# GaryGky/IDEAL-NeRF

Hardware: AMD Instinct MI355X
Metric: ray-samples/sec (64+128 pts, 512x512), whole job (higher is better)
Workload: dtype f32

## Files before the change

ideal-nerf_amd/csrc/idn_internal.h:

```cpp
#pragma once
#include <hip/hip_runtime.h>
#include <mutex>
#include <stdint.h>
#include <stddef.h>
#include "../../include/idealnerf.h"

namespace idn {

constexpr int kFragBytes = 1024;
constexpr int kFragFloats = 256;
constexpr int kSliceFrags = 64;
constexpr int kRingSlots = 2;
constexpr int kRingFrags = kRingSlots * kSliceFrags;
constexpr int kSliceBytes = kSliceFrags * kFragBytes;

constexpr int kNumLayers = 12;
constexpr int kLayerNT[kNumLayers] = {8, 8, 8, 8, 8, 8, 8, 8, 5, 4, 4, 1};
constexpr int kLayerKG[kNumLayers] = {8, 32, 32, 32, 32, 40, 32, 32, 36, 16, 16, 16};

constexpr int layer_f0(int l) {
    int f = 0;
    for (int i = 0; i < l; ++i) f += kLayerNT[i] * kLayerKG[i];
    return f;
}
constexpr int kUsedFrags = layer_f0(kNumLayers);
constexpr int kNumSlices =
    ((kUsedFrags + kSliceFrags - 1) / kSliceFrags + kRingSlots - 1) / kRingSlots * kRingSlots;
constexpr int kStreamFrags = kNumSlices * kSliceFrags;
static_assert(kUsedFrags == 2244, "layer table changed");
static_assert(kNumSlices % kRingSlots == 0, "slot of a slice must be static across passes");
static_assert(kRingFrags == 128, "FragReader addresses the ring as two 64-fragment halves");

constexpr int plain_f0(int l) {
    int f = 0;
    for (int i = 0; i < l; ++i) f += kLayerNT[i] * (kLayerKG[i] / 2);
    return f;
}
constexpr int kPlainUsedFrags = plain_f0(kNumLayers);
constexpr int kPlainNumSlices =
    ((kPlainUsedFrags + kSliceFrags - 1) / kSliceFrags + kRingSlots - 1) / kRingSlots * kRingSlots;
constexpr int kPlainStreamFrags = kPlainNumSlices * kSliceFrags;
static_assert(kPlainUsedFrags == 1122 && kPlainUsedFrags % 2 == 0, "plain stream table changed");

constexpr int kX6KFrags = 3;
constexpr int kX6SliceFrags = 16 * kX6KFrags;
constexpr int kX6RingFrags = kRingSlots * kX6SliceFrags;
constexpr int kX6UsedFrags = kX6KFrags * kPlainUsedFrags;
constexpr int kX6NumSlices = 2 * kNumSlices;
constexpr int kX6StreamFrags = kX6NumSlices * kX6SliceFrags;
static_assert(kX6UsedFrags <= kX6StreamFrags && kX6StreamFrags - kX6UsedFrags < kX6RingFrags + kX6SliceFrags, "x6 stream table");

constexpr int bias_off(int l) {
    int o = 0;
    for (int i = 0; i < l; ++i) o += kLayerNT[i] * 32;
    return o;
}
constexpr int kAlphaOff = bias_off(kNumLayers);
constexpr int kRgbOff = kAlphaOff + 256;
constexpr int kBiasFloats = kRgbOff + 3 * 128;
static_assert(kBiasFloats == 3136, "bias table changed");

constexpr int kSigmaChannel = 128;

enum { kActX0 = 0, kActDir = 1, kActA1 = 2, kActV1 = 10, kActCount = 13 };
constexpr int act_width(int i) { return i < 2 ? 64 : (i < kActV1 ? 256 : 128); }
constexpr int act_off(int i) {
    int o = 0;
    for (int k = 0; k < i; ++k) o += act_width(k);
    return o;
}
constexpr int kActCols = act_off(kActCount);
static_assert(kActCols == 2560, "activation slab layout changed");
constexpr int kMaskLayers = 11;
constexpr int kMaskFloatsPerPoint = kMaskLayers * 8;
constexpr int kActColsAll = kActCols + kMaskFloatsPerPoint;
__host__ __device__ inline size_t mask_index(int id, int64_t p_pad, int64_t wave_tile, int lane) {
    return ((size_t)id * (size_t)(p_pad / 32) + (size_t)wave_tile) * 64 + (size_t)lane;
}

int fail(int code, const char* fmt, ...);
#define IDN_HIP_CHECK(expr)                                                                   \
    do {                                                                                      \
        hipError_t _e = (expr);                                                               \
        if (_e != hipSuccess) return ::idn::fail(IDN_EHIP, "%s: %s", #expr, hipGetErrorString(_e)); \
    } while (0)

struct LaunchSetup {
    static constexpr int kMaxDevices = 64;
    std::mutex mu;
    int cus[kMaxDevices] = {};
    template <class OptIn>
    int get(OptIn&& opt_in, int* num_cu) {
        int dev = 0;
        IDN_HIP_CHECK(hipGetDevice(&dev));
        if (dev < 0 || dev >= kMaxDevices) return ::idn::fail(IDN_EUNSUPPORTED, "device index %d out of range", dev);
        std::lock_guard<std::mutex> lock(mu);
        if (!cus[dev]) {
            hipDeviceProp_t prop;
            IDN_HIP_CHECK(hipGetDeviceProperties(&prop, dev));
            if (int e = opt_in()) return e;
            cus[dev] = prop.multiProcessorCount;
        }
        *num_cu = cus[dev];
        return IDN_OK;
    }
};

struct ProfScope {
    int slot;
    hipStream_t s;
    ProfScope(hipStream_t s, int64_t points, int kind = IDN_PROF_MLP_FWD);
    ~ProfScope();
};

int launch_pack_f32(const idn_facenerf_params& p, float* packed, hipStream_t s);
int launch_pack_bf16x3(const idn_facenerf_params& p, float* packed, hipStream_t s, int fmt = 0);
int launch_pack_bf16x6(const idn_facenerf_params& p, float* packed, hipStream_t s);
int launch_mlp_bf16x6(const float* packed, const float* folded, const float* x, const float* rays, const float* z,
                      const float* pts, const float* dirs, int64_t n_points, int n_samples, float* raw, hipStream_t s,
                      float* acts = nullptr, int64_t p_pad = 0);
int launch_pack_bf16(const idn_facenerf_params& p, float* packed, hipStream_t s);
int launch_mlp_bf16(const float* packed, const float* folded, const float* x, const float* rays, const float* z,
                    const float* pts, const float* dirs, int64_t n_points, int n_samples, float* raw, hipStream_t s);
int launch_mlp_bf16x3(const float* packed, const float* folded, const float* x, const float* rays, const float* z,
                      const float* pts, const float* dirs, int64_t n_points, int n_samples, float* raw, hipStream_t s);
int launch_mlp_fp16x3(const float* packed, const float* folded, const float* x, const float* rays, const float* z,
                      const float* pts, const float* dirs, int64_t n_points, int n_samples, float* raw, hipStream_t s);
int launch_mlp(int precision, const float* packed, const float* folded, const float* x, const float* rays,
               const float* z, const float* pts, const float* dirs, int64_t n_points, int n_samples, float* raw,
               hipStream_t s);
int launch_fold(const idn_facenerf_params& p, const float* aud, const float* expr, const float* latent,
                float* folded, hipStream_t s);
int launch_mlp_f32(const float* packed, const float* folded, const float* x, const float* rays, const float* z,
                   const float* pts, const float* dirs, int64_t n_points, int n_samples, float* raw, hipStream_t s,
                   float* acts = nullptr, int64_t p_pad = 0);

int launch_frame_rays(const float* c2w, int H, int W, float focal, float cx, float cy, float near_, float far_,
                      int row0, int nrows, float* rays_out, hipStream_t s);
int launch_frame_rays_pixels(const float* c2w_host, int H, int W, float focal, float cx, float cy, float near_, float far_,
                             int64_t pix0, int npix, float* rays_out, hipStream_t s);
size_t audio_net_saved_floats(int n);
int launch_audio_net_fwd(const idn_audio_net_params* p, const float* windows, int n, float* out, float* saved, hipStream_t s);
int launch_audio_net_bwd(const idn_audio_net_params* p, const idn_audio_net_grads* g, const float* windows, const float* saved,
                         const float* d_out, int n, hipStream_t s);
int launch_to8b(const float* rgb, int64_t n_pixels, int swap_rb, unsigned char* out, int* flag, hipStream_t s);
int launch_compose_to8b(const float* head, const float* lw, const float* fg, int64_t n_pixels, int swap_rb,
                        unsigned char* out, unsigned char* fg_out, int* flag, hipStream_t s);
struct Draws {
    unsigned long long seed;
    long ray0;
    int on;
};
int launch_philox_uniform(unsigned long long seed, int which, int64_t row0, int64_t n_rows, int n_cols, float* out, hipStream_t s);
int launch_coarse_depths(const float* rays, const float* t_vals, const float* t_rand, int64_t n_rays, int S,
                         int lindisp, float* z, hipStream_t s, Draws draws = Draws{0, 0, 0});
int launch_composite(const float* raw, const float* z, const float* rays, const float* bc, int64_t n_rays, int S,
                     const float* noise, int white_bkgd, const idn_composite_out& out, hipStream_t s);
int launch_march(const float* raw, const float* z, const float* rays, const float* bc, const float* noise, int white_bkgd,
                 const idn_composite_out& out, const float* u, int u_per_ray, int64_t n_rays, int S, int Ni,
                 float* z_samples, int64_t* inds, float* cdf_out, float* z_fine, float* z_std, hipStream_t s,
                 Draws draws = Draws{0, 0, 0});
int launch_render_fused(int arrangement, const float* packed_c, const float* folded_c, const float* packed_f, const float* folded_f,
                        const float* rays, const float* bc, const float* z_c, float* z_f, const float* u, int u_per_ray, int64_t n_rays,
                        int white_bkgd, const idn_composite_out& co, const idn_composite_out& fo, float* z_std, float* tap_raw_c,
                        float* tap_raw_f, float* tap_z_fine, int64_t* tap_inds, float* tap_z_samples, float* tap_cdf, hipStream_t s,
                        Draws draws = Draws{0, 0, 0});
int launch_sample_pdf(const float* z, const float* weights, const float* cdf_in, const float* bins_in,
                      const float* u, int u_per_ray, int64_t n_rays, int S, int Ni, float* z_samples,
                      int64_t* inds, float* cdf_out, float* z_fine, float* z_std, hipStream_t s);

constexpr int kBwdStages = 11;
constexpr int kBwdNT[kBwdStages] = {4, 4, 4, 8, 8, 8, 8, 8, 8, 8, 8};
constexpr int kBwdKG[kBwdStages] = {2, 16, 16, 18, 32, 32, 32, 32, 32, 32, 32};
constexpr int kBwdHeadFrags = 280, kBwdTrunk0 = 384;
constexpr int bwd_f0(int s) {
    if (s >= 4) return kBwdTrunk0 + 256 * (s - 4);
    int f = 0;
    for (int i = 0; i < s; ++i) f += kBwdNT[i] * kBwdKG[i];
    return f;
}
static_assert(bwd_f0(3) + kBwdNT[3] * kBwdKG[3] == kBwdHeadFrags, "head stages");
constexpr int kBwdStreamFrags = kBwdTrunk0 + 7 * 256;
static_assert(kBwdStreamFrags % kSliceFrags == 0 && kBwdTrunk0 % kRingFrags == 0, "ring phase of the trunk stages");
constexpr int kBwdNumSlices = kBwdStreamFrags / kSliceFrags;

int launch_pack_f32_bwd(const idn_facenerf_params& p, float* packed_bwd, hipStream_t s);
int launch_delta_chain(const float* packed_bwd, const float* acts, int64_t p_pad, const float* d_rgb, float* dv0,
                       float* dv2, float* dv1, float* const da[8], hipStream_t s);
size_t bwd_stream_floats_x6();
int launch_pack_bf16x6_bwd(const idn_facenerf_params& p, float* packed_bwd, hipStream_t s);
int launch_delta_chain_x6(const float* packed_bwd, const float* acts, int64_t p_pad, const float* d_rgb, float* dv0,
                          float* dv2, float* dv1, float* const da[8], hipStream_t s);
size_t bwd_workspace_bytes(int64_t n_points);
size_t dw_gemm_workspace_bytes();
int launch_dw_gemm(const float* delta, int ld_delta, const float* acts, int ld_acts, int64_t rows, float* dW, float* db, int pipe,
                   void* ws, size_t ws_bytes, hipStream_t s);
int launch_pass_bwd(const idn_facenerf_params& p, const idn_facenerf_grads& gr, const float* aud, const float* expr,
                    const float* latent, const float* acts, const float* raw, const float* z, const float* rays,
                    const float* bc, int64_t n_rays, int S, const float* g_rgb, const float* g_fg, const float* g_lw,
                    const float* g_acc, float* d_aud, float* d_latent, void* ws, size_t ws_bytes, hipStream_t s);
int launch_facenerf_bwd(const idn_facenerf_params& p, const idn_facenerf_grads& gr, const float* aud, const float* expr,
                        const float* latent, const float* acts, int64_t n, const float* g_out, float* d_x, float* d_aud,
                        float* d_expr, float* d_latent, void* ws, size_t ws_bytes, hipStream_t s);

}
```

ideal-nerf_amd/csrc/mlp_f32_bwd.hip:

```cpp
#include "mlp_x6.h"

namespace idn {

__device__ __forceinline__ f32x16 mfma_b(float a, float b, f32x16 c) {
    return __builtin_amdgcn_mfma_f32_32x32x2f32(a, b, c, 0, 0, 0);
}

struct BwdPackStage {
    const float* w;
    const float* extra;
    int ld, col0, rows, cols, extra_at;
};
struct BwdPackDesc {
    BwdPackStage st[kBwdStages];
};
__global__ void pack_f32_bwd_kernel(BwdPackDesc d, float4* out) {
    const int gid = blockIdx.x * blockDim.x + threadIdx.x;
    if (gid >= kBwdStreamFrags * 64) return;
    const int f = gid >> 6, lane = gid & 63;
    float v[4] = {0.f, 0.f, 0.f, 0.f};
    int s = -1;
    for (int i = 0; i < kBwdStages; ++i)
        if (f >= bwd_f0(i) && f < bwd_f0(i) + kBwdNT[i] * kBwdKG[i]) s = i;
    if (s >= 0) {
        const BwdPackStage& S = d.st[s];
        const int rel = f - bwd_f0(s), t = rel / kBwdKG[s], g = rel - t * kBwdKG[s];
        const int n = 32 * t + (lane & 31);
        for (int j = 0; j < 4; ++j) {
            const int k = 8 * g + 4 * (lane >> 5) + j;
            if (n < S.cols) {
                if (k < S.rows) v[j] = S.w[(long)k * S.ld + S.col0 + n];
                else if (S.extra && k == S.extra_at) v[j] = S.extra[n];
            }
        }
    }
    out[gid] = make_float4(v[0], v[1], v[2], v[3]);
}

static void fill_bwd_desc(const idn_facenerf_params& p, BwdPackDesc& d) {
    const int C = p.dim_aud + p.dim_expr + p.dim_latent;
    d.st[0] = {p.rgb_w, nullptr, IDN_W / 2, 0, 3, IDN_W / 2, -1};
    d.st[1] = {p.views_w[2], nullptr, IDN_W / 2, 0, IDN_W / 2, IDN_W / 2, -1};
    d.st[2] = {p.views_w[1], nullptr, IDN_W / 2, 0, IDN_W / 2, IDN_W / 2, -1};
    d.st[3] = {p.views_w[0], p.alpha_w, IDN_W + IDN_VIEWS_CH + p.dim_expr, 0, IDN_W / 2, IDN_W, kSigmaChannel};
    for (int l = 7; l >= 1; --l) {
        BwdPackStage& S = d.st[4 + (7 - l)];
        S = {p.pts_w[l], nullptr, l == 5 ? IDN_PTS_CH + C + IDN_W : IDN_W, l == 5 ? IDN_PTS_CH + C : 0, IDN_W, IDN_W, -1};
    }
}

int launch_pack_f32_bwd(const idn_facenerf_params& p, float* packed_bwd, hipStream_t s) {
    BwdPackDesc d;
    fill_bwd_desc(p, d);
    const int total = kBwdStreamFrags * 64;
    hipLaunchKernelGGL(pack_f32_bwd_kernel, dim3((total + 255) / 256), dim3(256), 0, s, d, reinterpret_cast<float4*>(packed_bwd));
    IDN_HIP_CHECK(hipGetLastError());
    return IDN_OK;
}

struct DeltaArgs {
    const float* wstream;
    const float* acts;
    long p_pad;
    const float* d_rgb;
    float* dv0;
    float* dv2;
    float* dv1;
    float* da[8];
};

template <int F0, int NT, int KG, bool LAST, class BGet, class Side>
__device__ __forceinline__ void run_stage(f32x16 (&out)[NT], BGet&& bget, WStream& ws, FragReader& fr, Side&& side) {
    constexpr int STEPS = KG / 2, NP = NT * STEPS;
    static_assert(KG % 2 == 0 && F0 % 2 == 0, "fragments are consumed in pairs");
    if constexpr (F0 % kSliceFrags == 0) {
        ws.open_slice();
        fr.pref0 = fr.template issue<F0>();
        fr.pref1 = fr.template issue<F0 + 1>();
    }
    f32x4 a0 = fr.pref0, a1 = fr.pref1;
    static_for<NP>([&](auto PI) {
        constexpr int pi = decltype(PI)::value;
        constexpr int t = pi / STEPS, s = pi % STEPS, g0 = 2 * s, g1 = g0 + 1;
        constexpr int f = F0 + 2 * pi;
        constexpr bool next_crosses = ((f + 2) % kSliceFrags == 0);
        f32x4 n0 = a0, n1 = a1;
        if constexpr (!next_crosses && !(LAST && pi + 1 == NP)) {
            n0 = fr.template issue<f + 2>();
            n1 = fr.template issue<f + 3>();
            FragReader::retire<2>(a0, a1);
        } else {
            FragReader::retire<0>(a0, a1);
        }
        ws.template step_piece<f>();
        side(ic<t>{}, ic<s>{}, ic<0>{});
        out[t] = mfma_b(a0.x, bget(ic<g0>{}, ic<0>{}), out[t]);
        out[t] = mfma_b(a0.y, bget(ic<g0>{}, ic<1>{}), out[t]);
        out[t] = mfma_b(a0.z, bget(ic<g0>{}, ic<2>{}), out[t]);
        out[t] = mfma_b(a0.w, bget(ic<g0>{}, ic<3>{}), out[t]);
        out[t] = mfma_b(a1.x, bget(ic<g1>{}, ic<0>{}), out[t]);
        out[t] = mfma_b(a1.y, bget(ic<g1>{}, ic<1>{}), out[t]);
        out[t] = mfma_b(a1.z, bget(ic<g1>{}, ic<2>{}), out[t]);
        out[t] = mfma_b(a1.w, bget(ic<g1>{}, ic<3>{}), out[t]);
        if constexpr (next_crosses && pi + 1 < NP) {
            ws.open_slice();
            n0 = fr.template issue<f + 2>();
            n1 = fr.template issue<f + 3>();
        }
        a0 = n0;
        a1 = n1;
    });
    fr.pref0 = a0;
    fr.pref1 = a1;
}

template <int NT, int STEPS, int LD>
struct MaskSide {
    static constexpr bool kShadowStore = STEPS >= 8;
    f32x16* out;
    const uint32_t* mk;
    __amdgpu_buffer_rsrc_t rsrc;
    uint32_t voff;
    float* stage;
    float* rb;
    uint32_t raddr;
    int m, h;
    template <int T>
    __device__ __forceinline__ void apply(ic<T>) const {
        const uint32_t w = mk[T >> 1];
        static_for<16>([&](auto R) {
            constexpr int r = decltype(R)::value, i = 16 * (T & 1) + r;
            const int off = (int)(w << i) >> 31;
            out[T][r] = __uint_as_float(__float_as_uint(out[T][r]) & ~(uint32_t)off);
        });
    }
    template <int T>
    __device__ __forceinline__ void scatter(ic<T>) const {
        static_for<16>([&](auto R) {
            constexpr int r = decltype(R)::value;
            stage[m * kStagePitch + (r & 3) + 8 * (r >> 2) + 4 * h] = out[T][r];
        });
        asm volatile("" ::: "memory");
    }
    template <int Q>
    __device__ __forceinline__ void rows_read(ic<Q>) const {
        static_for<4>([&](auto I) {
            constexpr int i = decltype(I)::value;
            asm volatile("ds_read_b32 %0, %1 offset:%2" : "=v"(rb[i]) : "v"(raddr), "n"(2 * (4 * Q + i) * kStagePitch * 4) : "memory");
        });
    }
    template <int T, int Q>
    __device__ __forceinline__ void rows_store(ic<T>, ic<Q>) const {
        asm volatile("" : "+v"(rb[0]), "+v"(rb[1]), "+v"(rb[2]), "+v"(rb[3]));
        static_for<4>([&](auto I) {
            constexpr int i = decltype(I)::value;
            __builtin_amdgcn_raw_buffer_store_b32(__builtin_bit_cast(unsigned, rb[i]), rsrc, voff, (2 * (4 * Q + i) * LD + 32 * T) * 4, 0);
        });
    }
    template <int T>
    __device__ __forceinline__ void flush_tile(ic<T>) const {
        scatter(ic<T>{});
        static_for<4>([&](auto Q) {
            rows_read(Q);
            asm volatile("s_waitcnt lgkmcnt(0)" : "+v"(rb[0]), "+v"(rb[1]), "+v"(rb[2]), "+v"(rb[3])::"memory");
            rows_store(ic<T>{}, Q);
        });
    }
    __device__ __forceinline__ void finish() const {
        apply(ic<NT - 1>{});
        if constexpr (kShadowStore) flush_tile(ic<NT - 1>{});
        else static_for<NT>([&](auto T) { flush_tile(T); });
    }
    template <int T, int S, int H>
    __device__ __forceinline__ void operator()(ic<T>, ic<S>, ic<H>) const {
        constexpr int kApplyStep = STEPS > 1 ? 1 : 0;
        if constexpr (S == kApplyStep && T > 0) apply(ic<T - 1>{});
        if constexpr (kShadowStore && T > 0) {
            if constexpr (S == 2) scatter(ic<T - 1>{});
            if constexpr (S >= 4 && S <= 7) rows_store(ic<T - 1>{}, ic<S - 4>{});
            if constexpr (S >= 3 && S <= 6) rows_read(ic<S - 3>{});
        }
    }
};

template <int NT>
__device__ __forceinline__ void zero_tiles(f32x16 (&t)[NT]) {
    static_for<NT>([&](auto T) {
        static_for<16>([&](auto R) { t[decltype(T)::value][decltype(R)::value] = 0.0f; });
    });
}

constexpr int kDeltaLds = kRingFrags * kFragBytes + 4 * kStageFloats * 4;

__global__ __launch_bounds__(256, 1) void delta_chain_kernel(DeltaArgs a) {
    extern __shared__ __attribute__((aligned(16))) char smem[];
    char* ring = smem;
    const int tid = threadIdx.x, lane = tid & 63;
    const int wave = __builtin_amdgcn_readfirstlane(tid >> 6);
    const int m = lane & 31, h = lane >> 5;
    float* stage = reinterpret_cast<float*>(smem + kRingFrags * kFragBytes) + wave * kStageFloats;

    WStream ws;
    ws.init(a.wstream, kBwdNumSlices, ring, tid, wave);
    FragReader fr;
    fr.addr0 = (uint32_t)(uintptr_t)(__attribute__((address_space(3))) char*)ring + lane * 16;
    fr.addr1 = fr.addr0 + 64 * kFragBytes;
    const long ntiles = a.p_pad >> 7;
    const uint32_t raddr = (uint32_t)(uintptr_t)(__attribute__((address_space(3))) float*)stage + (h * kStagePitch + m) * 4;

    for (long tile = blockIdx.x; tile < ntiles; tile += gridDim.x) {
        const long p0 = tile * 128 + wave * 32;
        const long P = p0 + m;
        const f32x4 drgb = *reinterpret_cast<const f32x4*>(a.d_rgb + P * 64);
        const float dsig = a.dv0[P * 256 + kSigmaChannel];

        f32x16 A[8], B[8];
        float rb[4];
        typedef uint32_t u32x4 __attribute__((ext_vector_type(4)));
        const u32x4* mbase = reinterpret_cast<const u32x4*>(a.acts + (size_t)kActCols * a.p_pad);
        auto mask_load = [&](int id) { return mbase[mask_index(id, a.p_pad, tile * 4 + wave, lane)]; };
        u32x4 mask_nxt = mask_load(10);
        auto tiles_get = [](f32x16* arr) {
            return [arr](auto G, auto J) {
                constexpr int g = decltype(G)::value, j = decltype(J)::value;
                return arr[g >> 2][(g & 3) * 4 + j];
            };
        };
        auto stage_run = [&](auto Sc, auto F0c, auto LASTc, auto LDc, auto& out, auto&& bget, int next_id, float* dst) {
            constexpr int S = decltype(Sc)::value, F0 = decltype(F0c)::value;
            constexpr int NT = kBwdNT[S], KG = kBwdKG[S];
            zero_tiles<NT>(out);
            constexpr int LD = decltype(LDc)::value;
            const u32x4 mv = mask_nxt;
            const uint32_t mk[4] = {mv.x, mv.y, mv.z, mv.w};
            if (next_id >= 0) mask_nxt = mask_load(next_id);
            const MaskSide<NT, KG / 2, LD> side{&out[0], mk, rows_rsrc(dst + p0 * LD, LD), (uint32_t)((h * LD + m) * 4), stage, rb, raddr, m, h};
            run_stage<F0, NT, KG, decltype(LASTc)::value != 0>(out, bget, ws, fr, side);
            side.finish();
        };
        f32x16(&A4)[4] = reinterpret_cast<f32x16(&)[4]>(A);
        f32x16(&B4)[4] = reinterpret_cast<f32x16(&)[4]>(B);

        stage_run(ic<0>{}, ic<bwd_f0(0)>{}, ic<0>{}, ic<256>{}, A4,
                  [&](auto G, auto J) {
                      constexpr int g = decltype(G)::value, j = decltype(J)::value;
                      if constexpr (g == 0 && j < 3) return h ? 0.0f : drgb[j];
                      else return 0.0f;
                  },
                  9, a.dv2);
        stage_run(ic<1>{}, ic<bwd_f0(1)>{}, ic<0>{}, ic<256>{}, B4, tiles_get(A), 8, a.dv1);
        stage_run(ic<2>{}, ic<bwd_f0(2)>{}, ic<0>{}, ic<256>{}, A4, tiles_get(B), 7, a.dv0);
        stage_run(ic<3>{}, ic<bwd_f0(3)>{}, ic<1>{}, ic<256>{}, B,
                  [&](auto G, auto J) {
                      constexpr int g = decltype(G)::value, j = decltype(J)::value;
                      if constexpr (g < 16) return A[g >> 2][(g & 3) * 4 + j];
                      else if constexpr (g == 16 && j == 0) return h ? 0.0f : dsig;
                      else return 0.0f;
                  },
                  6, a.da[7]);
        finish_pass<kBwdHeadFrags, kBwdTrunk0>(ws);
#pragma unroll 1
        for (int l = 7; l >= 3; l -= 2) {
            stage_run(ic<4>{}, ic<bwd_f0(4)>{}, ic<0>{}, ic<256>{}, A, tiles_get(B), l - 2, a.da[l - 1]);
            stage_run(ic<5>{}, ic<bwd_f0(5)>{}, ic<0>{}, ic<256>{}, B, tiles_get(A), l - 3, a.da[l - 2]);
        }
        stage_run(ic<10>{}, ic<bwd_f0(10)>{}, ic<1>{}, ic<256>{}, A, tiles_get(B), -1, a.da[0]);
    }
    __builtin_amdgcn_s_waitcnt(0);
    __syncthreads();
}

int launch_delta_chain(const float* packed_bwd, const float* acts, int64_t p_pad, const float* d_rgb, float* dv0,
                       float* dv2, float* dv1, float* const da[8], hipStream_t s) {
    if (p_pad <= 0) return IDN_OK;
    if (p_pad % 128) return fail(IDN_EINVAL, "delta chain: p_pad %lld is not a multiple of 128", (long long)p_pad);
    static LaunchSetup setup;
    int num_cu = 0;
    if (int e = setup.get([]() -> int {
            IDN_HIP_CHECK(hipFuncSetAttribute(reinterpret_cast<const void*>(&delta_chain_kernel),
                                              hipFuncAttributeMaxDynamicSharedMemorySize, kDeltaLds));
            return IDN_OK;
        }, &num_cu))
        return e;
    const int64_t ntiles = p_pad / 128;
    const int grid = (int)(ntiles < num_cu ? ntiles : num_cu);
    DeltaArgs a{packed_bwd, acts, (long)p_pad, d_rgb, dv0, dv2, dv1, {}};
    for (int l = 0; l < 8; ++l) a.da[l] = da[l];
    ProfScope prof(s, p_pad, IDN_PROF_DELTA_CHAIN);
    hipLaunchKernelGGL(delta_chain_kernel, dim3(grid), dim3(256), kDeltaLds, s, a);
    IDN_HIP_CHECK(hipGetLastError());
    return IDN_OK;
}


constexpr int bwd6_f0(int s) { return kX6KFrags * (bwd_f0(s) / 2); }
constexpr int kBwd6StreamFrags = kX6KFrags * (kBwdStreamFrags / 2);
constexpr int kBwd6NumSlices = kBwd6StreamFrags / kX6SliceFrags;
static_assert(kBwd6StreamFrags % kX6SliceFrags == 0 && kBwd6NumSlices % kRingSlots == 0 && bwd6_f0(4) % kX6RingFrags == 0, "ring phase of the trunk stages");

__global__ void pack_bf16x6_bwd_kernel(BwdPackDesc d, uint4* out) {
    const int gid = blockIdx.x * blockDim.x + threadIdx.x;
    if (gid >= kBwd6StreamFrags * 64) return;
    const int f = gid >> 6, lane = gid & 63, part = f % kX6KFrags;
    unsigned w[4] = {0u, 0u, 0u, 0u};
    int s = -1;
    for (int i = 0; i < kBwdStages; ++i)
        if (f >= bwd6_f0(i) && f < bwd6_f0(i) + kX6KFrags * kBwdNT[i] * (kBwdKG[i] / 2)) s = i;
    if (s >= 0) {
        const BwdPackStage& S = d.st[s];
        const int ksn = kBwdKG[s] / 2;
        const int rel = (f - bwd6_f0(s)) / kX6KFrags, t = rel / ksn, ks = rel - t * ksn;
        const int n = 32 * t + (lane & 31), h = lane >> 5;
        for (int j = 0; j < 8; ++j) {
            const int k = 16 * ks + (j & 3) + 8 * (j >> 2) + 4 * h;
            float v = 0.f;
            if (n < S.cols) {
                if (k < S.rows) v = S.w[(long)k * S.ld + S.col0 + n];
                else if (S.extra && k == S.extra_at) v = S.extra[n];
            }
            const unsigned u1 = __float_as_uint(v);
            const unsigned p1 = (u1 + 0x7fffu + ((u1 >> 16) & 1u)) >> 16;
            const float r1 = v - __uint_as_float(p1 << 16);
            const unsigned u2 = __float_as_uint(r1);
            const unsigned p2 = (u2 + 0x7fffu + ((u2 >> 16) & 1u)) >> 16;
            const float r2 = r1 - __uint_as_float(p2 << 16);
            const unsigned u3 = __float_as_uint(r2);
            const unsigned p3 = (u3 + 0x7fffu + ((u3 >> 16) & 1u)) >> 16;
            const unsigned bits = part == 0 ? p1 : (part == 1 ? p2 : p3);
            w[j >> 1] |= bits << (16 * (j & 1));
        }
    }
    out[gid] = make_uint4(w[0], w[1], w[2], w[3]);
}

static_assert(kBwd6StreamFrags >= kBwdStreamFrags, "the six-piece stream is the larger of the two");
size_t bwd_stream_floats_x6() { return (size_t)kBwd6StreamFrags * kFragFloats; }

int launch_pack_bf16x6_bwd(const idn_facenerf_params& p, float* packed_bwd, hipStream_t s) {
    BwdPackDesc d;
    fill_bwd_desc(p, d);
    const int total = kBwd6StreamFrags * 64;
    hipLaunchKernelGGL(pack_bf16x6_bwd_kernel, dim3((total + 255) / 256), dim3(256), 0, s, d, reinterpret_cast<uint4*>(packed_bwd));
    IDN_HIP_CHECK(hipGetLastError());
    return IDN_OK;
}

namespace x6 {

template <int F0, int NT, int KS, bool LAST, int OPEN_YOUNGER, int MID_YOUNGER, class BGet, class Side>
__device__ __forceinline__ void run_stage6(f32x16* O, BGet&& bget, WStream6& ws, FragReader& fr, f32x4 (&pref)[3], Side&& side) {
    constexpr int NP = NT * KS;
    static_assert(F0 % kX6KFrags == 0, "triples");
    static_for<NT>([&](auto T) { static_for<16>([&](auto R) { O[decltype(T)::value][decltype(R)::value] = 0.0f; }); });
    if constexpr (F0 % kX6SliceFrags == 0) {
        ws.template open_slice<OPEN_YOUNGER>();
        static_for<3>([&](auto Q) { pref[decltype(Q)::value] = issue6<F0 + decltype(Q)::value>(fr); });
        retire3<0>(pref);
    }
    f32x4 a[3] = {pref[0], pref[1], pref[2]};
    static_for<NP>([&](auto PI) {
        constexpr int pi = decltype(PI)::value;
        constexpr int t = pi / KS, s = pi % KS;
        constexpr int f = F0 + kX6KFrags * pi;
        constexpr bool next_crosses = ((f + kX6KFrags) % kX6SliceFrags == 0);
        constexpr bool has_next = !(LAST && pi + 1 == NP);
        f32x4 n[3] = {a[0], a[1], a[2]};
        if constexpr (!next_crosses && has_next) {
            static_for<3>([&](auto Q) { n[decltype(Q)::value] = issue6<f + kX6KFrags + decltype(Q)::value>(fr); });
            if constexpr (pi > 0) retire3<3>(a);
        } else {
            if constexpr (pi > 0) retire3<0>(a);
        }
        step_pieces6<f>(ws);
        const f32x4 b1 = bget(ic<0>{}, ic<s>{}), b2 = bget(ic<1>{}, ic<s>{}), b3 = bget(ic<2>{}, ic<s>{});
        O[t] = mfma_bf(a[0], b1, O[t]);
        O[t] = mfma_bf(a[0], b2, O[t]);
        O[t] = mfma_bf(a[1], b1, O[t]);
        O[t] = mfma_bf(a[1], b2, O[t]);
        side(ic<t>{}, ic<s>{});
        O[t] = mfma_bf(a[0], b3, O[t]);
        O[t] = mfma_bf(a[2], b1, O[t]);
        if constexpr (next_crosses && pi + 1 < NP) {
            ws.template open_slice<(t >= 1 ? MID_YOUNGER : 0)>();
            static_for<3>([&](auto Q) { n[decltype(Q)::value] = issue6<f + kX6KFrags + decltype(Q)::value>(fr); });
        }
        a[0] = n[0];
        a[1] = n[1];
        a[2] = n[2];
    });
    if constexpr (!LAST && (F0 + kX6KFrags * NP) % kX6SliceFrags != 0) retire3<0>(a);
    pref[0] = a[0];
    pref[1] = a[1];
    pref[2] = a[2];
}

template <int KS>
struct MaskStoreSide {
    f32x16* O;
    const uint32_t* mk;
    float* row;
    template <int T>
    __device__ __forceinline__ void apply(ic<T>) const {
        const uint32_t w = mk[T >> 1];
        static_for<16>([&](auto R) {
            constexpr int r = decltype(R)::value, i = 16 * (T & 1) + r;
            const int off = (int)(w << i) >> 31;
            O[T][r] = __uint_as_float(__float_as_uint(O[T][r]) & ~(uint32_t)off);
        });
    }
    template <int T, int Q0>
    __device__ __forceinline__ void store2(ic<T>, ic<Q0>) const {
        static_for<2>([&](auto I) {
            constexpr int q = Q0 + decltype(I)::value;
            *reinterpret_cast<f32x4*>(row + 32 * T + 8 * q) = f32x4{O[T][4 * q], O[T][4 * q + 1], O[T][4 * q + 2], O[T][4 * q + 3]};
        });
    }
    template <int T>
    __device__ __forceinline__ void whole(ic<T>) const {
        apply(ic<T>{});
        store2(ic<T>{}, ic<0>{});
        store2(ic<T>{}, ic<2>{});
    }
    template <int T, int Q>
    __device__ __forceinline__ void store1(ic<T>, ic<Q>) const {
        *reinterpret_cast<f32x4*>(row + 32 * T + 8 * Q) = f32x4{O[T][4 * Q], O[T][4 * Q + 1], O[T][4 * Q + 2], O[T][4 * Q + 3]};
    }
    template <int T, int S>
    __device__ __forceinline__ void operator()(ic<T>, ic<S>) const {
        if constexpr (KS == 16 && T > 0) {
            if constexpr (S == 7) apply(ic<T - 1>{});
            if constexpr (S >= 8 && S < 16 && (S & 1) == 0) store1(ic<T - 1>{}, ic<(S - 8) / 2>{});
        }
    }
};

constexpr int kDelta6Lds = kX6RingFrags * kFragBytes;

__global__ __launch_bounds__(256, 1) void delta_chain_x6_kernel(DeltaArgs a) {
    extern __shared__ __attribute__((aligned(16))) char smem[];
    char* ring = smem;
    const int tid = threadIdx.x, lane = tid & 63;
    const int wave = __builtin_amdgcn_readfirstlane(tid >> 6);
    const int m = lane & 31, h = lane >> 5;

    WStream6 ws;
    ws.init(a.wstream, kBwd6NumSlices, ring, tid, wave);
    FragReader fr;
    fr.addr0 = (uint32_t)(uintptr_t)(__attribute__((address_space(3))) char*)ring + lane * 16;
    fr.addr1 = fr.addr0 + 64 * kFragBytes;
    const long ntiles = a.p_pad >> 7;
    f32x4 pref[3] = {{0.f, 0.f, 0.f, 0.f}, {0.f, 0.f, 0.f, 0.f}, {0.f, 0.f, 0.f, 0.f}};

    for (long tile = blockIdx.x; tile < ntiles; tile += gridDim.x) {
        const long P = tile * 128 + wave * 32 + m;
        const f32x4 drgb = *reinterpret_cast<const f32x4*>(a.d_rgb + P * 64);
        const float dsig = a.dv0[P * 256 + kSigmaChannel];
        f32x4 in_rgb[3], in_sig[3];
        {
            const f32x4 z4 = {0.f, 0.f, 0.f, 0.f};
            float r[3][2], g[3];
            split3(h ? 0.0f : drgb[0], h ? 0.0f : drgb[1], r[0][0], r[1][0], r[2][0]);
            split3(h ? 0.0f : drgb[2], 0.0f, r[0][1], r[1][1], r[2][1]);
            float unused0, unused1, unused2;
            (void)unused0; (void)unused1; (void)unused2;
            split3(h ? 0.0f : dsig, 0.0f, g[0], g[1], g[2]);
            static_for<3>([&](auto Q) {
                constexpr int q = decltype(Q)::value;
                in_rgb[q] = z4;
                in_rgb[q][0] = r[q][0];
                in_rgb[q][1] = r[q][1];
                in_sig[q] = z4;
                in_sig[q][0] = g[q];
            });
        }

        settle(in_rgb);
        settle(in_sig);
        PTile6 Pt[8];
        f32x16 O[8];
        typedef uint32_t u32x4 __attribute__((ext_vector_type(4)));
        const u32x4* mbase = reinterpret_cast<const u32x4*>(a.acts + (size_t)kActCols * a.p_pad);
        auto mask_load = [&](int id) { return mbase[mask_index(id, a.p_pad, tile * 4 + wave, lane)]; };
        u32x4 mask_nxt = mask_load(10);
        auto tiles = [&](auto Q, auto S_) {
            constexpr int q = decltype(Q)::value, s = decltype(S_)::value;
            return Pt[s >> 1].p[q][s & 1];
        };
        auto stage_run = [&](auto F0c, auto NTc, auto KSc, auto LASTc, auto LDc, auto YOUNGERc, auto&& bget, int next_id, float* dst) __attribute__((always_inline)) {
            constexpr int NT = decltype(NTc)::value, LD = decltype(LDc)::value;
            const u32x4 mv = mask_nxt;
            const uint32_t mk[4] = {mv.x, mv.y, mv.z, mv.w};
            if (next_id >= 0) mask_nxt = mask_load(next_id);
            const MaskStoreSide<decltype(KSc)::value> side{O, mk, dst + P * LD + 4 * h};
            constexpr bool trunk = decltype(F0c)::value >= bwd6_f0(4);
            run_stage6<decltype(F0c)::value, NT, decltype(KSc)::value, decltype(LASTc)::value != 0, decltype(YOUNGERc)::value, (trunk ? 4 : 0)>(O, bget, ws, fr, pref, side);
            if constexpr (trunk) side.whole(ic<NT - 1>{});
            else static_for<NT>([&](auto T) { side.whole(T); });
            static_for<NT>([&](auto T) { convert_tile<false>(O[decltype(T)::value], Pt[decltype(T)::value]); });
        };
        stage_run(ic<bwd6_f0(0)>{}, ic<4>{}, ic<1>{}, ic<0>{}, ic<256>{}, ic<0>{}, [&](auto Q, auto) { return in_rgb[decltype(Q)::value]; }, 9, a.dv2);
        stage_run(ic<bwd6_f0(1)>{}, ic<4>{}, ic<8>{}, ic<0>{}, ic<256>{}, ic<0>{}, tiles, 8, a.dv1);
        stage_run(ic<bwd6_f0(2)>{}, ic<4>{}, ic<8>{}, ic<0>{}, ic<256>{}, ic<0>{}, tiles, 7, a.dv0);
        stage_run(ic<bwd6_f0(3)>{}, ic<8>{}, ic<9>{}, ic<1>{}, ic<256>{}, ic<0>{},
                  [&](auto Q, auto S_) {
                      constexpr int q = decltype(Q)::value, s = decltype(S_)::value;
                      if constexpr (s < 8) return Pt[s >> 1].p[q][s & 1];
                      else return in_sig[q];
                  },
                  6, a.da[7]);
        finish_pass6<kX6KFrags * (kBwdHeadFrags / 2), bwd6_f0(4)>(ws);
        stage_run(ic<bwd6_f0(4)>{}, ic<8>{}, ic<16>{}, ic<0>{}, ic<256>{}, ic<0>{}, tiles, 5, a.da[6]);
#pragma unroll 1
        for (int L = 6; L >= 2; --L)
            stage_run(ic<bwd6_f0(5)>{}, ic<8>{}, ic<16>{}, ic<0>{}, ic<256>{}, ic<8>{}, tiles, L - 2, a.da[L - 1]);
        stage_run(ic<bwd6_f0(10)>{}, ic<8>{}, ic<16>{}, ic<1>{}, ic<256>{}, ic<8>{}, tiles, -1, a.da[0]);
    }
    __builtin_amdgcn_s_waitcnt(0);
    __syncthreads();
}

}

int launch_delta_chain_x6(const float* packed_bwd, const float* acts, int64_t p_pad, const float* d_rgb, float* dv0,
                          float* dv2, float* dv1, float* const da[8], hipStream_t s) {
    if (p_pad <= 0) return IDN_OK;
    if (p_pad % 128) return fail(IDN_EINVAL, "delta chain: p_pad %lld is not a multiple of 128", (long long)p_pad);
    static LaunchSetup setup;
    int num_cu = 0;
    if (int e = setup.get([]() -> int {
            IDN_HIP_CHECK(hipFuncSetAttribute(reinterpret_cast<const void*>(&x6::delta_chain_x6_kernel),
                                              hipFuncAttributeMaxDynamicSharedMemorySize, x6::kDelta6Lds));
            return IDN_OK;
        }, &num_cu))
        return e;
    const int64_t ntiles = p_pad / 128;
    const int grid = (int)(ntiles < num_cu ? ntiles : num_cu);
    DeltaArgs a{packed_bwd, acts, (long)p_pad, d_rgb, dv0, dv2, dv1, {}};
    for (int l = 0; l < 8; ++l) a.da[l] = da[l];
    ProfScope prof(s, p_pad, IDN_PROF_DELTA_CHAIN_X6);
    hipLaunchKernelGGL(x6::delta_chain_x6_kernel, dim3(grid), dim3(256), x6::kDelta6Lds, s, a);
    IDN_HIP_CHECK(hipGetLastError());
    return IDN_OK;
}

}
```

ideal-nerf_amd/csrc/train.hip:

```cpp
#include "idn_internal.h"
#include <cstdlib>
#include <type_traits>

namespace idn {

typedef float f32x16 __attribute__((ext_vector_type(16)));
typedef float f32x4 __attribute__((ext_vector_type(4)));

__device__ __forceinline__ f32x16 mfma32(float a, float b, f32x16 c) {
    return __builtin_amdgcn_mfma_f32_32x32x2f32(a, b, c, 0, 0, 0);
}
__device__ __forceinline__ int d_row(int r, int hh) { return (r & 3) + 8 * (r >> 2) + 4 * hh; }

struct TNArgs {
    const float* A; int lda;
    const float* B; int ldb;
    float* part;
    int N, K;
    long P;
    int chunks_per_split;
    float* cpart;
    int b_split, b_off0, b_off1;
};

template <int N>
struct LdsVec;
template <>
struct LdsVec<4> {
    f32x4 v;
    template <int OFF>
    __device__ __forceinline__ void issue(uint32_t addr) { asm volatile("ds_read_b128 %0, %1 offset:%2" : "=v"(v) : "v"(addr), "n"(OFF) : "memory"); }
    __device__ __forceinline__ float get(int j) const { return v[j]; }
};
template <>
struct LdsVec<2> {
    typedef float f32x2 __attribute__((ext_vector_type(2)));
    f32x2 v;
    template <int OFF>
    __device__ __forceinline__ void issue(uint32_t addr) { asm volatile("ds_read_b64 %0, %1 offset:%2" : "=v"(v) : "v"(addr), "n"(OFF) : "memory"); }
    __device__ __forceinline__ float get(int j) const { return v[j]; }
};
template <>
struct LdsVec<1> {
    float v;
    template <int OFF>
    __device__ __forceinline__ void issue(uint32_t addr) { asm volatile("ds_read_b32 %0, %1 offset:%2" : "=v"(v) : "v"(addr), "n"(OFF) : "memory"); }
    __device__ __forceinline__ float get(int) const { return v; }
};
template <int OFF>
__device__ __forceinline__ void lds_read_f32(float& dst, uint32_t addr) {
    asm volatile("ds_read_b32 %0, %1 offset:%2" : "=v"(dst) : "v"(addr), "n"(OFF) : "memory");
}
__device__ __forceinline__ float landed(float& v) {
    asm volatile("" : "+v"(v));
    return v;
}
template <int NEWER, class VA, class VB>
__device__ __forceinline__ void lds_retire(VA& a, VB& b) {
    if constexpr (NEWER == 0) asm volatile("s_waitcnt lgkmcnt(0)" : "+v"(a.v), "+v"(b.v)::"memory");
    else asm volatile("s_waitcnt lgkmcnt(2)" : "+v"(a.v), "+v"(b.v)::"memory");
}
template <int N>
using ic_ = std::integral_constant<int, N>;
template <int N, class F>
__device__ __forceinline__ void tn_static_for(F&& f) {
    if constexpr (N > 0) {
        tn_static_for<N - 1>(f);
        f(std::integral_constant<int, N - 1>{});
    }
}

constexpr int kTnRows = 16, kTnBufs = 3;
constexpr int kTnNarrowBufs = 3;
constexpr int kTnRows4x1 = 32, kTnRowsThin = 64;
constexpr int kTnNarrowSplits = 256;

template <int NTW, int KTW, int NB = kTnBufs, int R = kTnRows>
__global__ __launch_bounds__(256) void gemm_tn_kernel(TNArgs g) {
    static_assert(R % 16 == 0, "chunks are multiples of 16 points");
    constexpr int NPA = NTW * R / 16, NPB = KTW * R / 16;
    static_assert(NB >= 3 && (NB - 2) * (NPA + NPB) <= 63, "vmcnt is a 6-bit field");
    constexpr int BN = 64 * NTW, BK = 64 * KTW;
    constexpr int kTileFloats = R * (BN + BK);
    constexpr int kSteps = R / 2;
    constexpr int NP = NPA + NPB;
    static_assert(NP <= kSteps, "at most one piece per step");
    extern __shared__ __attribute__((aligned(16))) float tn_smem[];
    const int tid = threadIdx.x, lane = tid & 63;
    const int w = __builtin_amdgcn_readfirstlane(tid >> 6);
    const int i = lane & 31, hh = lane >> 5;
    const int wr = w >> 1, wc = w & 1;
    const int n0 = blockIdx.x * BN, k0 = blockIdx.y * BK;
    const int split = blockIdx.z;
    f32x16 acc[NTW][KTW];
#pragma unroll
    for (int a = 0; a < NTW; ++a)
#pragma unroll
        for (int b = 0; b < KTW; ++b)
            for (int r = 0; r < 16; ++r) acc[a][b][r] = 0.f;

    const long c_begin = (long)split * g.chunks_per_split;
    long c_end = c_begin + g.chunks_per_split;
    const long c_total = g.P / R;
    if (c_end > c_total) c_end = c_total;
    const bool colsum_block = g.cpart != nullptr && blockIdx.y == 0;
    const bool do_colsum = colsum_block && tid < BN;
    const int ccol = tid < BN ? tid : 0;
    float csum = 0.0f;

    constexpr int kRowsPerPieceA = 256 / BN > 0 ? 256 / BN : 1, kRowsPerPieceB = 256 / BK > 0 ? 256 / BK : 1;
    const __amdgpu_buffer_rsrc_t rsrcA = __builtin_amdgcn_make_buffer_rsrc(const_cast<float*>(g.A + n0 + c_begin * R * (long)g.lda), 0, 0xfffffffc, 0x00020000);
    const __amdgpu_buffer_rsrc_t rsrcB = __builtin_amdgcn_make_buffer_rsrc(const_cast<float*>(g.B + k0 + c_begin * R * (long)g.ldb), 0, 0xfffffffc, 0x00020000);
    const uint32_t voffA = ((lane / (BN / 4)) * g.lda + (lane % (BN / 4)) * 4) * 4;
    const uint32_t voffB = ((lane / (BK / 4)) * g.ldb + (lane % (BK / 4)) * 4) * 4;
    const uint32_t rowA = g.lda * 4, rowB = g.ldb * 4;
    auto piece_a = [&](long c, int buf, int ja) {
        const int pc = NPA * w + ja;
        __builtin_amdgcn_raw_ptr_buffer_load_lds(rsrcA, (__attribute__((address_space(3))) void*)(tn_smem + buf * kTileFloats + pc * 256), 16, voffA,
                                                 (uint32_t)(((c - c_begin) * R + pc * kRowsPerPieceA) * rowA), 0, 0);
    };
    auto piece_b = [&](long c, int buf, int jb) {
        const int pc = NPB * w + jb;
        __builtin_amdgcn_raw_ptr_buffer_load_lds(rsrcB, (__attribute__((address_space(3))) void*)(tn_smem + buf * kTileFloats + R * BN + pc * 256), 16, voffB,
                                                 (uint32_t)(((c - c_begin) * R + pc * kRowsPerPieceB) * rowB), 0, 0);
    };
    auto piece = [&](long c, int buf, int j) {
        if (j < NPA) piece_a(c, buf, j);
        else if (j < NP) piece_b(c, buf, j - NPA);
    };
    const uint32_t smem0 = (uint32_t)(uintptr_t)(__attribute__((address_space(3))) float*)tn_smem;
    const uint32_t a_addr0 = smem0 + (hh * BN + NTW * (32 * wr + i)) * 4;
    const uint32_t b_addr0 = smem0 + (R * BN + hh * BK + KTW * (32 * wc + i)) * 4;
    for (int ahead = 0; ahead < NB - 1; ++ahead)
        for (int j = 0; j < NP; ++j) piece(c_begin + ahead < c_end ? c_begin + ahead : c_end - 1, ahead, j);
    int buf = 0;
    for (long c = c_begin; c < c_end; ++c) {
        asm volatile("s_waitcnt vmcnt(%0)" ::"n"((NB - 2) * NP) : "memory");
        __builtin_amdgcn_s_barrier();
        asm volatile("" ::: "memory");
        const int buf2 = buf >= 1 ? buf - 1 : NB - 1;
        const long cnext = c + NB - 1 < c_end ? c + NB - 1 : c_end - 1;
        float cs[16];
        auto cs_issue = [&](int batch) {
            const uint32_t caddr = smem0 + buf * (kTileFloats * 4) + ccol * 4 + batch * (16 * BN * 4);
            tn_static_for<16>([&](auto Row) {
                lds_read_f32<decltype(Row)::value * BN * 4>(cs[decltype(Row)::value], caddr);
            });
        };
        static_assert(R / 16 <= kSteps / 4, "one batch of column reads per iteration of the first half loop");
        if (colsum_block) cs_issue(0);
        LdsVec<NTW> a0v, a1v;
        LdsVec<KTW> b0v, b1v;
        constexpr int kStepA = 2 * BN * 4, kStepB = 2 * BK * 4;
        uint32_t pa = a_addr0 + buf * (kTileFloats * 4), pb = b_addr0 + buf * (kTileFloats * 4);
        a0v.template issue<0>(pa);
        b0v.template issue<0>(pb);
        static_assert(NPA <= kSteps / 2 && NPB <= kSteps / 2, "pieces of one matrix fit one half of a chunk");
        constexpr int M = NTW * KTW;
        if constexpr (M >= 4) {
            auto step = [&](LdsVec<NTW>& ca, LdsVec<KTW>& cb, auto&& side0, auto&& side1, auto&& side2) {
                lds_retire<0>(ca, cb);
                tn_static_for<M>([&](auto M_) {
                    constexpr int m = decltype(M_)::value, x = m / KTW, y = m % KTW;
                    acc[x][y] = mfma32(ca.get(x), cb.get(y), acc[x][y]);
                    if constexpr (m < 3) {
                        __builtin_amdgcn_sched_barrier(0);
                        if constexpr (m == 0) side0();
                        if constexpr (m == 1) side1();
                        if constexpr (m == 2) side2();
                        __builtin_amdgcn_sched_barrier(0);
                    }
                });
            };
#pragma unroll 1
            for (int it = 0; it < kSteps / 4; ++it) {
                step(a0v, b0v,
                     [&]() { a1v.template issue<kStepA>(pa); b1v.template issue<kStepB>(pb); },
                     [&]() { if (2 * it < NPA) piece_a(cnext, buf2, 2 * it); },
                     [&]() {
                         if (colsum_block && it < R / 16) {
                             tn_static_for<16>([&](auto Row) { csum += landed(cs[decltype(Row)::value]); });
                         }
                         pa += 2 * kStepA;
                         pb += 2 * kStepB;
                     });
                step(a1v, b1v,
                     [&]() { a0v.template issue<0>(pa); b0v.template issue<0>(pb); },
                     [&]() { if (2 * it + 1 < NPA) piece_a(cnext, buf2, 2 * it + 1); },
                     [&]() { if (colsum_block && it + 1 < R / 16) cs_issue(it + 1); });
            }
#pragma unroll 1
            for (int it = 0; it < kSteps / 4; ++it) {
                const bool last = it == kSteps / 4 - 1;
                step(a0v, b0v,
                     [&]() { a1v.template issue<kStepA>(pa); b1v.template issue<kStepB>(pb); },
                     [&]() { if (2 * it < NPB) piece_b(cnext, buf2, 2 * it); },
                     [&]() {
                         pa = last ? pa : pa + 2 * kStepA;
                         pb = last ? pb : pb + 2 * kStepB;
                     });
                step(a1v, b1v,
                     [&]() { a0v.template issue<0>(pa); b0v.template issue<0>(pb); },
                     [&]() { if (2 * it + 1 < NPB) piece_b(cnext, buf2, 2 * it + 1); },
                     [&]() {});
            }
        } else {
            static_assert(M == 2 && kSteps % 8 == 0, "the two-pair schedule");
            LdsVec<NTW> a2v, a3v;
            LdsVec<KTW> b2v, b3v;
            a1v.template issue<kStepA>(pa);
            b1v.template issue<kStepB>(pb);
            auto quad = [&](LdsVec<NTW>& c0a, LdsVec<KTW>& c0b, LdsVec<NTW>& c1a, LdsVec<KTW>& c1b, LdsVec<NTW>& n0a, LdsVec<KTW>& n0b,
                            LdsVec<NTW>& n1a, LdsVec<KTW>& n1b, bool last, auto&& side_c, auto&& side_d) {
                lds_retire<0>(c0a, c0b);
                lds_retire<0>(c1a, c1b);
                const uint32_t na = last ? pa : pa + 2 * kStepA, nb = last ? pb : pb + 2 * kStepB;
                auto mf = [&](LdsVec<NTW>& ca, LdsVec<KTW>& cb, auto M_) {
                    constexpr int m = decltype(M_)::value, x = m / KTW, y = m % KTW;
                    acc[x][y] = mfma32(ca.get(x), cb.get(y), acc[x][y]);
                    __builtin_amdgcn_sched_barrier(0);
                };
                mf(c0a, c0b, ic_<0>{});
                n0a.template issue<0>(na);
                n0b.template issue<0>(nb);
                __builtin_amdgcn_sched_barrier(0);
                mf(c0a, c0b, ic_<1>{});
                n1a.template issue<kStepA>(na);
                n1b.template issue<kStepB>(nb);
                __builtin_amdgcn_sched_barrier(0);
                mf(c1a, c1b, ic_<0>{});
                side_c();
                __builtin_amdgcn_sched_barrier(0);
                mf(c1a, c1b, ic_<1>{});
                side_d();
                pa = na;
                pb = nb;
                __builtin_amdgcn_sched_barrier(0);
            };
#pragma unroll 1
            for (int it = 0; it < kSteps / 8; ++it) {
                quad(a0v, b0v, a1v, b1v, a2v, b2v, a3v, b3v, false,
                     [&]() { if (2 * it < NPA) piece_a(cnext, buf2, 2 * it); },
                     [&]() {
                         if (colsum_block && it < R / 16) {
                             tn_static_for<16>([&](auto Row) { csum += landed(cs[decltype(Row)::value]); });
                         }
                     });
                quad(a2v, b2v, a3v, b3v, a0v, b0v, a1v, b1v, false,
                     [&]() { if (2 * it + 1 < NPA) piece_a(cnext, buf2, 2 * it + 1); },
                     [&]() { if (colsum_block && it + 1 < R / 16) cs_issue(it + 1); });
            }
#pragma unroll 1
            for (int it = 0; it < kSteps / 8; ++it) {
                quad(a0v, b0v, a1v, b1v, a2v, b2v, a3v, b3v, false,
                     [&]() { if (2 * it < NPB) piece_b(cnext, buf2, 2 * it); }, [&]() {});
                quad(a2v, b2v, a3v, b3v, a0v, b0v, a1v, b1v, it == kSteps / 8 - 1,
                     [&]() { if (2 * it + 1 < NPB) piece_b(cnext, buf2, 2 * it + 1); }, [&]() {});
            }
            lds_retire<0>(a1v, b1v);
        }
        lds_retire<0>(a0v, b0v);
        buf = buf + 1 == NB ? 0 : buf + 1;
    }
    asm volatile("s_waitcnt vmcnt(0)" ::: "memory");
    if (do_colsum) g.cpart[(long)split * g.N + n0 + tid] = csum;
    float* out = g.part + (long)split * g.N * g.K;
#pragma unroll
    for (int x = 0; x < NTW; ++x)
#pragma unroll
        for (int r = 0; r < 16; ++r) {
            const int n = n0 + NTW * (32 * wr + d_row(r, hh)) + x;
            float* dst = out + (long)n * g.K + k0 + KTW * (32 * wc + i);
            if constexpr (KTW == 4) {
                *reinterpret_cast<f32x4*>(dst) = f32x4{acc[x][0][r], acc[x][1][r], acc[x][2][r], acc[x][3][r]};
            } else {
#pragma unroll
                for (int y = 0; y < KTW; ++y) dst[y] = acc[x][y][r];
            }
        }
}

typedef __bf16 tn_bf16x8 __attribute__((ext_vector_type(8)));
typedef unsigned tn_u32x4 __attribute__((ext_vector_type(4)));
typedef int tn_i32x4 __attribute__((ext_vector_type(4)));
__device__ __forceinline__ f32x16 mfma_bf16(f32x4 a, f32x4 b, f32x16 c) {
    return __builtin_amdgcn_mfma_f32_32x32x16_bf16(__builtin_bit_cast(tn_bf16x8, a), __builtin_bit_cast(tn_bf16x8, b), c, 0, 0, 0);
}
__device__ __forceinline__ unsigned tn_cvt_pk_bf16(float x0, float x1) {
    unsigned r;
    asm("v_cvt_pk_bf16_f32 %0, %1, %2" : "=v"(r) : "v"(x0), "v"(x1));
    return r;
}
__device__ __forceinline__ void split3(float x0, float x1, unsigned& p1, unsigned& p2, unsigned& p3) {
    p1 = tn_cvt_pk_bf16(x0, x1);
    float r0 = x0 - __uint_as_float(p1 << 16), r1 = x1 - __uint_as_float(p1 & 0xffff0000u);
    p2 = tn_cvt_pk_bf16(r0, r1);
    r0 = r0 - __uint_as_float(p2 << 16);
    r1 = r1 - __uint_as_float(p2 & 0xffff0000u);
    p3 = tn_cvt_pk_bf16(r0, r1);
}
constexpr int kX6BufBytes = 2 * 8 * 3 * kFragBytes;
constexpr int kX6Lds = 2 * kX6BufBytes;

struct X6Frag {
    f32x4 v;
    template <int OFF>
    __device__ __forceinline__ void issue(uint32_t addr) { asm volatile("ds_read_b128 %0, %1 offset:%2" : "=v"(v) : "v"(addr), "n"(OFF) : "memory"); }
};
template <int N>
__device__ __forceinline__ void x6_retire(X6Frag (&f)[3]) {
    static_assert(N <= 15, "lgkmcnt is a 4-bit field");
    asm volatile("s_waitcnt lgkmcnt(%3)" : "+v"(f[0].v), "+v"(f[1].v), "+v"(f[2].v) : "n"(N) : "memory");
}

__device__ __forceinline__ void gemm_tn_x6_item(const TNArgs& g, const int split, char* x6_smem) {
    const int tid = threadIdx.x, lane = tid & 63;
    const int w = __builtin_amdgcn_readfirstlane(tid >> 6);
    const int i = lane & 31, hh = lane >> 5;
    const int wr = w >> 1, wc = w & 1;
    f32x16 acc[4][4];
#pragma unroll
    for (int a = 0; a < 4; ++a)
#pragma unroll
        for (int b = 0; b < 4; ++b)
            for (int r = 0; r < 16; ++r) acc[a][b][r] = 0.f;

    const long c_begin = (long)split * g.chunks_per_split;
    long c_end = c_begin + g.chunks_per_split;
    const long c_total = g.P / kTnRows;
    if (c_end > c_total) c_end = c_total;
    const int n_chunks = (int)(c_end - c_begin);
    auto make_rsrc = [](const float* ptr) {
        const uint64_t a64 = (uint64_t)(uintptr_t)ptr;
        return tn_i32x4{(int)(uint32_t)a64, (int)((uint32_t)(a64 >> 32) & 0xffffu), (int)0xfffffffcu, 0x00020000};
    };
    const tn_i32x4 rsrcA = make_rsrc(g.A + c_begin * kTnRows * (long)g.lda);
    const tn_i32x4 rsrcB = make_rsrc(g.B + c_begin * kTnRows * (long)g.ldb);
    const int voff = tid * 4;
    const int voffB = g.b_split ? (tid < 128 ? g.b_off0 : g.b_off1) + (tid & 127) * 4 : voff;
    const int rowA = g.lda * 4, rowB = g.ldb * 4;
    float ra[kTnRows], rb[kTnRows];
#pragma unroll
    for (int p = 0; p < kTnRows; ++p) ra[p] = rb[p] = 0.f;
    auto load_row_at = [&](float& dst, const tn_i32x4& rsrc, int soff, int vo) {
        asm volatile("buffer_load_dword %0, %1, %2, %3 offen" : "+v"(dst) : "v"(vo), "s"(rsrc), "s"(soff) : "memory");
    };
    auto load_row = [&](float& dst, const tn_i32x4& rsrc, int soff) { load_row_at(dst, rsrc, soff, voff); };
    auto load_chunk = [&](int rc) {
        const int base = (rc < n_chunks ? rc : n_chunks - 1) * kTnRows;
#pragma unroll
        for (int p = 0; p < kTnRows; ++p) load_row(ra[p], rsrcA, (base + p) * rowA);
#pragma unroll
        for (int p = 0; p < kTnRows; ++p) load_row_at(rb[p], rsrcB, (base + p) * rowB, voffB);
    };
    char* const my_slot = x6_smem + (tid >> 5) * (3 * kFragBytes) + (tid & 31) * 16;
    auto split_store = [&](int buf, int X, const float (&r)[kTnRows]) {
        unsigned pw[3][8];
#pragma unroll
        for (int j = 0; j < 8; ++j) split3(r[2 * j], r[2 * j + 1], pw[0][j], pw[1][j], pw[2][j]);
        char* dst = my_slot + buf * kX6BufBytes + X * (8 * 3 * kFragBytes);
#pragma unroll
        for (int q = 0; q < 3; ++q)
#pragma unroll
            for (int h2 = 0; h2 < 2; ++h2)
                *reinterpret_cast<tn_u32x4*>(dst + q * kFragBytes + h2 * 512) =
                    tn_u32x4{pw[q][4 * h2], pw[q][4 * h2 + 1], pw[q][4 * h2 + 2], pw[q][4 * h2 + 3]};
    };
    const bool do_colsum = g.cpart != nullptr;
    float csum = 0.0f, csum1 = 0.0f;
    auto colsum = [&]() {
        float s0 = (ra[0] + ra[1]) + (ra[2] + ra[3]), s1 = (ra[4] + ra[5]) + (ra[6] + ra[7]);
        float s2 = (ra[8] + ra[9]) + (ra[10] + ra[11]), s3 = (ra[12] + ra[13]) + (ra[14] + ra[15]);
        csum += (s0 + s1) + (s2 + s3);
    };
    const uint32_t smem0 = (uint32_t)(uintptr_t)(__attribute__((address_space(3))) char*)x6_smem;
    const uint32_t a_base = smem0 + (4 * wr) * (3 * kFragBytes) + lane * 16;
    const uint32_t b_base = smem0 + (8 + 4 * wc) * (3 * kFragBytes) + lane * 16;

    load_chunk(0);
#pragma unroll
    for (int p = 0; p < kTnRows; ++p) asm volatile("s_waitcnt vmcnt(0)" : "+v"(ra[p]), "+v"(rb[p])::"memory");
    colsum();
    split_store(0, 0, ra);
    split_store(0, 1, rb);
    load_chunk(1);
    asm volatile("s_waitcnt lgkmcnt(0)" ::: "memory");
    __builtin_amdgcn_s_barrier();
    asm volatile("" ::: "memory");

    X6Frag fa[4][3], fb[4][3];
    auto issue_first_row = [&](uint32_t pa, uint32_t pb) {
        tn_static_for<3>([&](auto Q) { fa[0][decltype(Q)::value].template issue<decltype(Q)::value * kFragBytes>(pa); });
        tn_static_for<2>([&](auto Y) {
            tn_static_for<3>([&](auto Q) {
                fb[decltype(Y)::value][decltype(Q)::value].template issue<(decltype(Y)::value * 3 + decltype(Q)::value) * kFragBytes>(pb);
            });
        });
    };
    issue_first_row(a_base, b_base);
#pragma unroll 1
    for (int rc = 0; rc < n_chunks; ++rc) {
        const int buf = rc & 1;
        const uint32_t pa = a_base + buf * kX6BufBytes, pb = b_base + buf * kX6BufBytes;
        tn_static_for<2>([&](auto Y) {
            tn_static_for<3>([&](auto Q) {
                fb[decltype(Y)::value + 2][decltype(Q)::value].template issue<((decltype(Y)::value + 2) * 3 + decltype(Q)::value) * kFragBytes>(pb);
            });
        });
        tn_static_for<3>([&](auto X) {
            tn_static_for<3>([&](auto Q) {
                fa[decltype(X)::value + 1][decltype(Q)::value].template issue<((decltype(X)::value + 1) * 3 + decltype(Q)::value) * kFragBytes>(pa);
            });
        });
        auto mm2 = [&](int x, int y0, int y1) {
#define X6_TERM(QA, QB)                                                   \
    acc[x][y0] = mfma_bf16(fa[x][QA].v, fb[y0][QB].v, acc[x][y0]);        \
    acc[x][y1] = mfma_bf16(fa[x][QA].v, fb[y1][QB].v, acc[x][y1]);
            X6_TERM(0, 0) X6_TERM(0, 1) X6_TERM(1, 0) X6_TERM(1, 1) X6_TERM(0, 2) X6_TERM(2, 0)
#undef X6_TERM
        };
        x6_retire<15>(fa[0]);
        x6_retire<15>(fb[0]);
        x6_retire<15>(fb[1]);
        mm2(0, 0, 1);
        x6_retire<9>(fb[2]);
        x6_retire<9>(fb[3]);
        mm2(0, 2, 3);
        x6_retire<0>(fa[1]);
        x6_retire<0>(fa[2]);
        x6_retire<0>(fa[3]);
        const unsigned live_mask = rc + 1 < n_chunks ? 0xffffffffu : 0u;
        const int nbase = (rc + 2 < n_chunks ? rc + 2 : n_chunks - 1) * kTnRows;
        char* const dst = my_slot + (buf ^ 1) * kX6BufBytes;
        unsigned pw[2][3][8];
        float t0 = 0.f, t1 = 0.f;
        auto slice = [&](auto X_, auto S_) {
            constexpr int X = decltype(X_)::value, sl = decltype(S_)::value;
            float (&r)[kTnRows] = *(X ? &rb : &ra);
            auto store = [&](auto Q_, auto H_) {
                constexpr int q = decltype(Q_)::value, h2 = decltype(H_)::value;
                *reinterpret_cast<tn_u32x4*>(dst + X * (8 * 3 * kFragBytes) + q * kFragBytes + h2 * 512) =
                    tn_u32x4{pw[X][q][4 * h2], pw[X][q][4 * h2 + 1], pw[X][q][4 * h2 + 2], pw[X][q][4 * h2 + 3]};
            };
            if constexpr (sl < 24) {
                constexpr int j = sl / 3, ph = sl % 3;
                if constexpr (ph == 0) {
                    asm volatile("s_waitcnt vmcnt(30)" : "+v"(r[2 * j]), "+v"(r[2 * j + 1])::"memory");
                    const unsigned p1 = tn_cvt_pk_bf16(r[2 * j], r[2 * j + 1]);
                    pw[X][0][j] = p1;
                    t0 = r[2 * j] - __uint_as_float(p1 << 16);
                    t1 = r[2 * j + 1] - __uint_as_float(p1 & 0xffff0000u);
                    if constexpr (X == 0) {
                        csum += __uint_as_float(__float_as_uint(r[2 * j]) & live_mask);
                        csum1 += __uint_as_float(__float_as_uint(r[2 * j + 1]) & live_mask);
                        asm volatile("" : "+v"(csum), "+v"(csum1));
                    }
                } else if constexpr (ph == 1) {
                    const unsigned p2 = tn_cvt_pk_bf16(t0, t1);
                    pw[X][1][j] = p2;
                    t0 = t0 - __uint_as_float(p2 << 16);
                    t1 = t1 - __uint_as_float(p2 & 0xffff0000u);
                    pw[X][2][j] = tn_cvt_pk_bf16(t0, t1);
                } else {
                    load_row_at(r[2 * j], X ? rsrcB : rsrcA, (nbase + 2 * j) * (X ? rowB : rowA), X ? voffB : voff);
                    load_row_at(r[2 * j + 1], X ? rsrcB : rsrcA, (nbase + 2 * j + 1) * (X ? rowB : rowA), X ? voffB : voff);
                    if constexpr (j >= 3 && j < 6) store(ic_<j - 3>{}, ic_<0>{});
                    if constexpr (j == 7) store(ic_<0>{}, ic_<1>{});
                }
            } else if constexpr (sl == 24) {
                store(ic_<1>{}, ic_<1>{});
            } else if constexpr (sl == 25) {
                store(ic_<2>{}, ic_<1>{});
            }
        };
        __builtin_amdgcn_sched_barrier(0);
        tn_static_for<72>([&](auto K_) {
            constexpr int k = decltype(K_)::value;
            constexpr int x = 1 + k / 24, kk = k % 24, y = 2 * (kk / 12) + (kk % 2), t = (kk % 12) / 2;
            constexpr int qa = t == 2 || t == 3 ? 1 : (t == 5 ? 2 : 0);
            constexpr int qb = t == 1 || t == 3 ? 1 : (t == 4 ? 2 : 0);
            acc[x][y] = mfma_bf16(fa[x][qa].v, fb[y][qb].v, acc[x][y]);
            constexpr int kX1 = 26;
            if constexpr (k < kX1) slice(ic_<0>{}, ic_<k>{});
            else slice(ic_<1>{}, ic_<k - kX1>{});
            if constexpr (k == 59) {
                asm volatile("s_waitcnt lgkmcnt(0)" ::: "memory");
                __builtin_amdgcn_s_barrier();
                asm volatile("" ::: "memory");
                issue_first_row(a_base + (buf ^ 1) * kX6BufBytes, b_base + (buf ^ 1) * kX6BufBytes);
            }
            __builtin_amdgcn_sched_barrier(0);
        });
    }
    x6_retire<0>(fa[0]);
    x6_retire<0>(fb[0]);
    x6_retire<0>(fb[1]);
#pragma unroll
    for (int p = 0; p < kTnRows; ++p) asm volatile("s_waitcnt vmcnt(0)" : "+v"(ra[p]), "+v"(rb[p])::"memory");
    if (do_colsum) g.cpart[(long)split * g.N + tid] = csum + csum1;
    float* out = g.part + (long)split * g.N * g.K;
#pragma unroll
    for (int x = 0; x < 4; ++x)
#pragma unroll
        for (int y = 0; y < 4; ++y)
#pragma unroll
            for (int r = 0; r < 16; ++r)
                out[(long)(32 * (4 * wr + x) + d_row(r, hh)) * g.K + 32 * (4 * wc + y) + i] = acc[x][y][r];
}
constexpr int kMaxTnBatch = 12;
struct TNBatch {
    TNArgs it[kMaxTnBatch];
    int n, splits;
};
__global__ __launch_bounds__(256) void gemm_tn_x6_kernel(TNBatch b) {
    extern __shared__ __attribute__((aligned(16))) char x6_smem[];
    const int item = __builtin_amdgcn_readfirstlane((int)blockIdx.z / b.splits);
    const int split = __builtin_amdgcn_readfirstlane((int)blockIdx.z - item * b.splits);
    gemm_tn_x6_item(b.it[item], split, x6_smem);
}

constexpr int kMaxReduceItems = 32;
struct ReduceItem {
    const float* part;
    float* out;
    int splits, N, K, ldo, rows, cols;
    int block_end;
};
struct ReduceBatch {
    ReduceItem it[kMaxReduceItems];
    int n;
};
__global__ __launch_bounds__(256) void reduce_batch_kernel(ReduceBatch b) {
    __shared__ double red[4][64];
    int i = 0;
    while (i + 1 < b.n && (int)blockIdx.x >= b.it[i].block_end) ++i;
    const ReduceItem& t = b.it[i];
    const int block0 = i ? b.it[i - 1].block_end : 0;
    const int o = threadIdx.x & 63, q = threadIdx.x >> 6;
    const int idx = ((int)blockIdx.x - block0) * 64 + o;
    const bool live = idx < t.rows * t.cols;
    const int n = live ? idx / t.cols : 0, k = live ? idx % t.cols : 0;
    double s = 0.0;
    if (live) {
        const float* src = t.part + (long)n * t.K + k;
        const long stride = (long)t.N * t.K;
#pragma unroll 8
        for (int sp = q; sp < t.splits; sp += 4) s += (double)src[sp * stride];
    }
    red[q][o] = s;
    __syncthreads();
    if (q == 0 && live) t.out[(long)n * t.ldo + k] = (float)(((red[0][o] + red[1][o]) + red[2][o]) + red[3][o]);
}

__device__ __forceinline__ double shfl_up_dd(double v, int delta) {
    int lo = __double2loint(v), hi = __double2hiint(v);
    lo = __shfl_up(lo, delta, 64);
    hi = __shfl_up(hi, delta, 64);
    return __hiloint2double(hi, lo);
}
__device__ __forceinline__ double shfl_xor_dd(double v, int mask) {
    int lo = __double2loint(v), hi = __double2hiint(v);
    lo = __shfl_xor(lo, mask, 64);
    hi = __shfl_xor(hi, mask, 64);
    return __hiloint2double(hi, lo);
}

struct CompBwdArgs {
    const float4* raw; const float* z; const float* rays; const float* bc;
    const float* g_rgb;
    const float* g_fg;
    const float* g_lw;
    const float* g_acc;
    float* d_rgb; int ld_rgb;
    float* d_sig; int ld_sig;
    long n_rays; int S;
};

template <int SPL>
__global__ __launch_bounds__(256) void composite_bwd_kernel(CompBwdArgs a) {
    const int lane = threadIdx.x & 63;
    const long ray = (long)blockIdx.x * 4 + (threadIdx.x >> 6);
    if (ray >= a.n_rays) return;
    const int S = a.S;
    const float* rr = a.rays + ray * IDN_RAY_FLOATS;
    const float dn = sqrtf((rr[3] * rr[3] + rr[4] * rr[4]) + rr[5] * rr[5]);
    const float4* rawr = a.raw + ray * S;
    const float* zr = a.z + ray * S;
    float gr = 0, gg = 0, gb = 0, fr = 0, fg = 0, fb = 0, glw = 0, gacc = 0;
    if (a.g_rgb) { gr = a.g_rgb[ray * 3]; gg = a.g_rgb[ray * 3 + 1]; gb = a.g_rgb[ray * 3 + 2]; }
    if (a.g_fg) { fr = a.g_fg[ray * 3]; fg = a.g_fg[ray * 3 + 1]; fb = a.g_fg[ray * 3 + 2]; }
    if (a.g_lw) glw = a.g_lw[ray];
    if (a.g_acc) gacc = a.g_acc[ray];

    float zs[SPL + 1];
    float4 rw[SPL];
#pragma unroll
    for (int i = 0; i < SPL; ++i) {
        const int s = lane * SPL + i;
        zs[i] = s < S ? zr[s] : 0.f;
        rw[i] = s < S ? rawr[s] : make_float4(0.f, 0.f, 0.f, 0.f);
    }
    zs[SPL] = __shfl_down(zs[0], 1, 64);
    float alpha[SPL], tf[SPL], ex[SPL], dist[SPL];
    double local = 1.0;
#pragma unroll
    for (int i = 0; i < SPL; ++i) {
        const int s = lane * SPL + i;
        float d = (s >= S - 1) ? 1e10f : (zs[i + 1] - zs[i]);
        d = d * dn;
        const float e = expf(-(fmaxf(rw[i].w, 0.0f) + 1e-6f) * d);
        dist[i] = d;
        ex[i] = e;
        alpha[i] = (s < S) ? 1.0f - e : 0.0f;
        tf[i] = (s < S) ? (1.0f - (1.0f - e)) + 1e-10f : 1.0f;
        local *= (double)tf[i];
    }
    double incl = local;
#pragma unroll
    for (int d = 1; d < 64; d <<= 1) {
        const double o = shfl_up_dd(incl, d);
        if (lane >= d) incl *= o;
    }
    double run = shfl_up_dd(incl, 1);
    if (lane == 0) run = 1.0;
    float T[SPL], w[SPL], dw[SPL], cr[SPL], cg[SPL], cb[SPL];
    double lsum = 0.0;
#pragma unroll
    for (int i = 0; i < SPL; ++i) {
        const int s = lane * SPL + i;
        T[i] = (float)run;
        w[i] = alpha[i] * T[i];
        run *= (double)tf[i];
        dw[i] = 0.f;
        cr[i] = cg[i] = cb[i] = 0.f;
        if (s < S) {
            if (s == S - 1) {
                cr[i] = a.bc[ray * 3]; cg[i] = a.bc[ray * 3 + 1]; cb[i] = a.bc[ray * 3 + 2];
                dw[i] = (gr * cr[i] + gg * cg[i] + gb * cb[i]) + glw + gacc;
            } else {
                cr[i] = 1.0f / (1.0f + expf(-rw[i].x));
                cg[i] = 1.0f / (1.0f + expf(-rw[i].y));
                cb[i] = 1.0f / (1.0f + expf(-rw[i].z));
                dw[i] = ((gr + fr) * cr[i] + (gg + fg) * cg[i] + (gb + fb) * cb[i]) + gacc;
            }
            lsum += (double)dw[i] * (double)w[i];
        }
    }
    double pin = lsum;
#pragma unroll
    for (int d = 1; d < 64; d <<= 1) {
        const double o = shfl_up_dd(pin, d);
        if (lane >= d) pin += o;
    }
    double total = lsum;
#pragma unroll
    for (int m = 32; m >= 1; m >>= 1) total += shfl_xor_dd(total, m);
    double before = pin - lsum;
#pragma unroll
    for (int i = 0; i < SPL; ++i) {
        const int s = lane * SPL + i;
        if (s < S) {
            before += (double)dw[i] * (double)w[i];
            const double suffix = total - before;
            const float dalpha = dw[i] * T[i] - (float)(suffix / (double)tf[i]);
            const float dsig = (rw[i].w > 0.f) ? dalpha * ex[i] * dist[i] : 0.f;
            const long p = ray * S + s;
            a.d_sig[p * a.ld_sig] = dsig;
            float d0 = 0.f, d1 = 0.f, d2 = 0.f;
            if (s < S - 1) {
                d0 = w[i] * (gr + fr) * cr[i] * (1.0f - cr[i]);
                d1 = w[i] * (gg + fg) * cg[i] * (1.0f - cg[i]);
                d2 = w[i] * (gb + fb) * cb[i] * (1.0f - cb[i]);
            }
            a.d_rgb[p * a.ld_rgb + 0] = d0;
            a.d_rgb[p * a.ld_rgb + 1] = d1;
            a.d_rgb[p * a.ld_rgb + 2] = d2;
        }
    }
}

struct FoldBwdArgs {
    idn_facenerf_params p;
    const float* aud; const float* expr; const float* latent;
    const float* db0; const float* db5; const float* dbv;
    float* gW0; float* gW5; float* gWv0;
    float* d_aud; float* d_latent;
    float* d_expr;
};
__device__ __forceinline__ float cond_val(const FoldBwdArgs& d, int c) {
    if (c < d.p.dim_aud) return d.aud[c];
    c -= d.p.dim_aud;
    if (c < d.p.dim_expr) return d.expr[c] * 1.0f / 3.0f;
    c -= d.p.dim_expr;
    return d.latent[c];
}
__global__ void fold_bwd_kernel(FoldBwdArgs d) {
    const int C = d.p.dim_aud + d.p.dim_expr + d.p.dim_latent;
    const int ld0 = IDN_PTS_CH + C, ld5 = IDN_PTS_CH + C + IDN_W, ldv = IDN_W + IDN_VIEWS_CH + d.p.dim_expr;
    const int idx = blockIdx.x * blockDim.x + threadIdx.x;
    const int n_outer = IDN_W * C;
    if (idx < n_outer) {
        const int n = idx / C, c = idx % C;
        const float cv = cond_val(d, c);
        d.gW0[(long)n * ld0 + IDN_PTS_CH + c] = d.db0[n] * cv;
        d.gW5[(long)n * ld5 + IDN_PTS_CH + c] = d.db5[n] * cv;
    } else if (idx < n_outer + (IDN_W / 2) * d.p.dim_expr) {
        const int k = idx - n_outer, n = k / d.p.dim_expr, e = k % d.p.dim_expr;
        d.gWv0[(long)n * ldv + IDN_W + IDN_VIEWS_CH + e] = d.dbv[n] * (d.expr[e] * 1.0f / 3.0f);
    } else {
        const int rel = idx - n_outer - (IDN_W / 2) * d.p.dim_expr;
        const int c = rel >> 6, lane = rel & 63;
        if (c >= C) return;
        double s = 0.0;
        for (int n = lane; n < IDN_W; n += 64)
            s += (double)d.p.pts_w[0][(long)n * ld0 + IDN_PTS_CH + c] * (double)d.db0[n] +
                 (double)d.p.pts_w[5][(long)n * ld5 + IDN_PTS_CH + c] * (double)d.db5[n];
#pragma unroll
        for (int m = 32; m >= 1; m >>= 1) s += shfl_xor_dd(s, m);
        const int e = c - d.p.dim_aud;
        const bool want_expr = d.d_expr != nullptr && e >= 0 && e < d.p.dim_expr;
        double sv = 0.0;
        if (want_expr) {
            for (int n = lane; n < IDN_W / 2; n += 64)
                sv += (double)d.p.views_w[0][(long)n * ldv + IDN_W + IDN_VIEWS_CH + e] * (double)d.dbv[n];
#pragma unroll
            for (int m = 32; m >= 1; m >>= 1) sv += shfl_xor_dd(sv, m);
        }
        if (lane != 0) return;
        if (c < d.p.dim_aud) {
            if (d.d_aud) d.d_aud[c] += (float)s;
        } else if (c >= d.p.dim_aud + d.p.dim_expr) {
            if (d.d_latent) d.d_latent[c - d.p.dim_aud - d.p.dim_expr] += (float)s;
        } else if (want_expr) {
            d.d_expr[e] += (float)((s + sv) / 3.0);
        }
    }
}

static size_t al256(size_t x) { return (x + 255) & ~(size_t)255; }
constexpr int kMaxSplits = 256;
constexpr int kColsumBlocks = 256;
constexpr int kGemmsPerPass = 16;
constexpr int kX6ItemsPerPass = 9;
constexpr size_t kPartFloatsPerSplit = 9 * 65536 + 6 * 16384 + 4 * 8192;

struct BwdWs {
    float *dA[8], *dV[2], *dV0, *dRGB, *part, *cpart, *wbwd;
    size_t bytes;
};
static BwdWs carve_bwd(char* base, int64_t p_pad) {
    BwdWs w;
    size_t off = 0;
    auto take = [&](size_t floats) {
        float* p = reinterpret_cast<float*>(base + off);
        off += al256(floats * 4);
        return p;
    };
    for (int l = 0; l < 8; ++l) w.dA[l] = take((size_t)p_pad * 256);
    w.dV[0] = take((size_t)p_pad * 256);
    w.dV[1] = w.dV[0] + 128;
    w.dV0 = take((size_t)p_pad * 256);
    w.dRGB = take((size_t)p_pad * 64);
    w.part = take((size_t)kMaxSplits * kPartFloatsPerSplit);
    w.cpart = take((size_t)kColsumBlocks * 256 * kGemmsPerPass);
    w.wbwd = take(bwd_stream_floats_x6());
    w.bytes = off;
    return w;
}

size_t bwd_workspace_bytes(int64_t n_points) {
    const int64_t p_pad = (n_points + 127) / 128 * 128;
    return carve_bwd(nullptr, p_pad).bytes;
}

enum { kPipeX6 = 0, kPipeF32 = 1 };
static int env_pipe_f32() {
    static const int v = [] {
        const char* e = getenv("IDN_BACKWARD_PIPE");
        return (e && e[0] == 'f' && e[1] == '3' && e[2] == '2' && e[3] == 0) ? 1 : 0;
    }();
    return v;
}
static int default_gemm_pipe() { return env_pipe_f32() ? kPipeF32 : kPipeX6; }
struct X6Pending {
    TNBatch b;
    int splits = 0;
    int expected_items = 1;
    X6Pending() { b.n = 0; }
    int launch(hipStream_t s) {
        if (b.n == 0) return IDN_OK;
        static LaunchSetup setup6;
        int num_cu = 0;
        if (int e = setup6.get([]() -> int {
                IDN_HIP_CHECK(hipFuncSetAttribute(reinterpret_cast<const void*>(&gemm_tn_x6_kernel), hipFuncAttributeMaxDynamicSharedMemorySize, kX6Lds));
                return IDN_OK;
            }, &num_cu))
            return e;
        {
            ProfScope prof(s, b.it[0].P * b.n, IDN_PROF_DW_GEMM_X6);
            b.splits = splits;
            hipLaunchKernelGGL(gemm_tn_x6_kernel, dim3(1, 1, splits * b.n), dim3(256), kX6Lds, s, b);
        }
        IDN_HIP_CHECK(hipGetLastError());
        b.n = 0;
        return IDN_OK;
    }
    int add(const TNArgs& g, int item_splits, hipStream_t s) {
        if (b.n && (b.n == kMaxTnBatch || item_splits != splits || g.P != b.it[0].P))
            if (int e = launch(s)) return e;
        splits = item_splits;
        b.it[b.n++] = g;
        return IDN_OK;
    }
};
static int device_cus(int* out) {
    static LaunchSetup st;
    return st.get([]() -> int { return IDN_OK; }, out);
}
template <int NTW, int KTW, int NB, int R = kTnRows>
static int launch_tn(const TNArgs& g, dim3 grid, hipStream_t s) {
    constexpr size_t lds = (size_t)NB * R * (size_t)(64 * NTW + 64 * KTW) * 4;
    static_assert(lds <= 160 * 1024, "the chunk ring must fit a CU's LDS");
    static LaunchSetup setup;
    int num_cu = 0;
    if (int e = setup.get([]() -> int {
            IDN_HIP_CHECK(hipFuncSetAttribute(reinterpret_cast<const void*>(&gemm_tn_kernel<NTW, KTW, NB, R>),
                                              hipFuncAttributeMaxDynamicSharedMemorySize, (int)lds));
            return IDN_OK;
        }, &num_cu))
        return e;
    hipLaunchKernelGGL((gemm_tn_kernel<NTW, KTW, NB, R>), grid, dim3(256), lds, s, g);
    IDN_HIP_CHECK(hipGetLastError());
    return IDN_OK;
}
static int run_tn_partials(X6Pending& x6, const float* A, int lda, int N, const float* B, int ldb, int K, int64_t P, float* part,
                           int* splits_out, hipStream_t s, float* cpart = nullptr, int pipe = -1, const float* B2 = nullptr) {
    if (pipe < 0) pipe = default_gemm_pipe();
    if (B2 && !(N == 256 && K == 256 && pipe == kPipeX6)) return fail(IDN_EINVAL, "gemm_tn: a split B needs the 256 x 256 bf16-piece kernel");
    int ntw, ktw;
    if (N == 256 && K == 256) { ntw = 4; ktw = 4; }
    else if (N == 256 && K == 64) { ntw = 4; ktw = 1; }
    else if (N == 128 && K == 256) { ntw = 2; ktw = 4; }
    else if (N == 128 && K == 64) { ntw = 2; ktw = 1; }
    else if (N == 128 && K == 128) { ntw = 2; ktw = 2; }
    else if (N == 64 && K == 128) { ntw = 1; ktw = 2; }
    else return fail(IDN_EUNSUPPORTED, "gemm_tn: no instantiation for %d x %d", N, K);
    const int bx = N / (64 * ntw), by = K / (64 * ktw);
    const bool narrow = ntw * ktw <= 4 && !(ntw == 2 && ktw == 2);
    const int rows_per_chunk = !narrow ? kTnRows : (ntw == 4 ? kTnRows4x1 : kTnRowsThin);
    if (P % rows_per_chunk) return fail(IDN_EINVAL, "gemm_tn: %lld rows are not a multiple of the %d-row chunk", (long long)P, rows_per_chunk);
    const long chunks = P / rows_per_chunk;
    int splits = (narrow ? kTnNarrowSplits : kMaxSplits) / (bx * by);
    if (ntw == 4 && ktw == 4 && pipe == kPipeX6) {
        int cus = 0;
        if (int e = device_cus(&cus)) return e;
        splits = 2 * cus / (x6.expected_items > 0 ? x6.expected_items : 1);
        if (splits > kMaxSplits) splits = kMaxSplits;
    }
    if (splits > chunks) splits = (int)chunks;
    if (splits < 1) splits = 1;
    const int cps = (int)((chunks + splits - 1) / splits);
    splits = (int)((chunks + cps - 1) / cps);
    TNArgs g{A, lda, B, ldb, part, N, K, (long)P, cps, cpart, 0, 0, 0};
    if (B2) {
        const float* base = B < B2 ? B : B2;
        const int64_t o0 = (int64_t)(B - base) * 4, o1 = (int64_t)(B2 - base) * 4;
        if (o0 >= (int64_t)1 << 31 || o1 >= (int64_t)1 << 31) return fail(IDN_EUNSUPPORTED, "gemm_tn: split B matrices more than 2 GiB apart");
        g.B = base;
        g.b_split = 1;
        g.b_off0 = (int)o0;
        g.b_off1 = (int)o1;
    }
    const dim3 grid(bx, by, splits);
    if (ntw == 4 && ktw == 4 && pipe == kPipeX6) {
        if (int e = x6.add(g, splits, s)) return e;
        *splits_out = splits;
        return IDN_OK;
    }
    ProfScope prof(s, P, IDN_PROF_DW_GEMM);
    int e;
    if (ntw == 4 && ktw == 4) e = launch_tn<4, 4, kTnBufs>(g, grid, s);
    else if (ntw == 4 && ktw == 1) e = launch_tn<4, 1, kTnNarrowBufs, kTnRows4x1>(g, grid, s);
    else if (ntw == 2 && ktw == 4) e = launch_tn<2, 4, kTnBufs>(g, grid, s);
    else if (ntw == 2 && ktw == 1) e = launch_tn<2, 1, kTnNarrowBufs, kTnRowsThin>(g, grid, s);
    else if (ntw == 2 && ktw == 2) e = launch_tn<2, 2, kTnBufs>(g, grid, s);
    else e = launch_tn<1, 2, kTnNarrowBufs, kTnRowsThin>(g, grid, s);
    if (e) return e;
    *splits_out = splits;
    return IDN_OK;
}
struct ReduceQueue {
    ReduceBatch b;
    int blocks = 0;
    float* part_next;
    float* cpart_next;
    X6Pending x6;
    ReduceQueue(float* part_pool, float* cpart_pool, int expected_x6_items = 1) : part_next(part_pool), cpart_next(cpart_pool) {
        b.n = 0;
        x6.expected_items = expected_x6_items;
    }
    int add(const float* part, int splits, int N, int K, int row0, int col0, float* out, int ldo, int rows, int cols) {
        if (b.n >= kMaxReduceItems) return fail(IDN_EUNSUPPORTED, "reduce queue full");
        blocks += (rows * cols + 63) / 64;
        b.it[b.n++] = ReduceItem{part + (size_t)row0 * K + col0, out, splits, N, K, ldo, rows, cols, blocks};
        return IDN_OK;
    }
    int flush(hipStream_t s) {
        if (int e = x6.launch(s)) return e;
        if (b.n == 0) return IDN_OK;
        hipLaunchKernelGGL(reduce_batch_kernel, dim3(blocks), dim3(256), 0, s, b);
        IDN_HIP_CHECK(hipGetLastError());
        b.n = 0;
        blocks = 0;
        return IDN_OK;
    }
};
static int run_tn_q(ReduceQueue& q, const float* A, int lda, int N, const float* B, int ldb, int K, int64_t P, int* splits,
                    const float** part_out, const float** cpart_out, bool colsum, hipStream_t s, int pipe, const float* B2 = nullptr) {
    float* part = q.part_next;
    float* cpart = colsum ? q.cpart_next : nullptr;
    if (int e = run_tn_partials(q.x6, A, lda, N, B, ldb, K, P, part, splits, s, cpart, pipe, B2)) return e;
    q.part_next += (size_t)(*splits) * N * K;
    if (colsum) q.cpart_next += (size_t)(*splits) * N;
    *part_out = part;
    if (cpart_out) *cpart_out = cpart;
    return IDN_OK;
}
static int run_tn(ReduceQueue& q, const float* A, int lda, int N, const float* B, int ldb, int K, int64_t P, float* out,
                  int ldo, int rows, int cols, hipStream_t s, float* db = nullptr, int db_cols = 0,
                  int pipe = -1) {
    int splits = 0;
    const float *part, *cpart;
    if (int e = run_tn_q(q, A, lda, N, B, ldb, K, P, &splits, &part, &cpart, db != nullptr, s, pipe)) return e;
    if (db)
        if (int e = q.add(cpart, splits, 1, N, 0, 0, db, N, 1, db_cols)) return e;
    return q.add(part, splits, N, K, 0, 0, out, ldo, rows, cols);
}

size_t dw_gemm_workspace_bytes() { return al256((size_t)kMaxSplits * 65536 * 4) + al256((size_t)kColsumBlocks * 256 * 4); }
int launch_dw_gemm(const float* delta, int ld_delta, const float* acts, int ld_acts, int64_t rows, float* dW, float* db, int pipe,
                   void* ws, size_t ws_bytes, hipStream_t s) {
    if (rows <= 0 || rows % 128) return fail(IDN_EINVAL, "dw_gemm: rows %lld is not a positive multiple of 128", (long long)rows);
    if (ld_delta < 256 || ld_acts < 256) return fail(IDN_EINVAL, "dw_gemm: row pitch < 256");
    const int as_in_a_pass = pipe == 2;
    if (as_in_a_pass) pipe = kPipeX6;
    if (pipe != kPipeX6 && pipe != kPipeF32) return fail(IDN_EINVAL, "dw_gemm: pipe %d", pipe);
    if (!ws || ws_bytes < dw_gemm_workspace_bytes()) return fail(IDN_EWORKSPACE, "dw_gemm workspace %zu < %zu", ws_bytes, dw_gemm_workspace_bytes());
    float* part = reinterpret_cast<float*>(ws);
    float* cpart = reinterpret_cast<float*>(reinterpret_cast<char*>(ws) + al256((size_t)kMaxSplits * 65536 * 4));
    ReduceQueue q(part, cpart, as_in_a_pass ? kX6ItemsPerPass : 1);
    if (int e = run_tn(q, delta, ld_delta, 256, acts, ld_acts, 256, rows, dW, 256, 256, 256, s, db, db ? 256 : 0, pipe)) return e;
    return q.flush(s);
}

static int bwd_tail(const idn_facenerf_params& p, const idn_facenerf_grads& gr, const float* aud, const float* expr,
                    const float* latent, const float* acts, int64_t Pp, const BwdWs& w, float* d_aud, float* d_expr,
                    float* d_latent, hipStream_t s) {
    const int C = p.dim_aud + p.dim_expr + p.dim_latent;
    const int ld0 = IDN_PTS_CH + C, ld5 = IDN_PTS_CH + C + IDN_W, ldv = IDN_W + IDN_VIEWS_CH + p.dim_expr;
    auto act = [&](int i) { return acts + (size_t)act_off(i) * Pp; };
    auto a_l = [&](int l) { return act(kActA1 + l - 1); };
    auto v_l = [&](int l) { return act(kActV1 + l - 1); };
#define TRY(x) do { if (int e_ = (x)) return e_; } while (0)
    if (!env_pipe_f32()) {
        TRY(launch_pack_bf16x6_bwd(p, w.wbwd, s));
        TRY(launch_delta_chain_x6(w.wbwd, acts, Pp, w.dRGB, w.dV0, w.dV[0], w.dV[1], w.dA, s));
    } else {
        TRY(launch_pack_f32_bwd(p, w.wbwd, s));
        TRY(launch_delta_chain(w.wbwd, acts, Pp, w.dRGB, w.dV0, w.dV[0], w.dV[1], w.dA, s));
    }
    ReduceQueue q(w.part, w.cpart, kX6ItemsPerPass);
    TRY(run_tn(q, w.dRGB, 64, 64, v_l(3), 128, 128, Pp, gr.rgb_w, 128, 3, 128, s, gr.rgb_b, 3));
    const int pipe = default_gemm_pipe();
    if (pipe == kPipeX6) {
        int splits = 0;
        const float *part, *cpart;
        TRY(run_tn_q(q, w.dV[0], 256, 256, v_l(2), 128, 256, Pp, &splits, &part, &cpart, true, s, pipe, v_l(1)));
        TRY(q.add(cpart, splits, 1, 256, 0, 0, gr.views_b[2], 128, 1, 128));
        TRY(q.add(cpart, splits, 1, 256, 0, 128, gr.views_b[1], 128, 1, 128));
        TRY(q.add(part, splits, 256, 256, 0, 0, gr.views_w[2], 128, 128, 128));
        TRY(q.add(part, splits, 256, 256, 128, 128, gr.views_w[1], 128, 128, 128));
    } else {
        TRY(run_tn(q, w.dV[0], 256, 128, v_l(2), 128, 128, Pp, gr.views_w[2], 128, 128, 128, s, gr.views_b[2], 128));
        TRY(run_tn(q, w.dV[1], 256, 128, v_l(1), 128, 128, Pp, gr.views_w[1], 128, 128, 128, s, gr.views_b[1], 128));
    }
    {
        int splits = 0;
        const float *part, *cpart;
        TRY(run_tn_q(q, w.dV0, 256, 256, a_l(8), 256, 256, Pp, &splits, &part, &cpart, true, s, pipe));
        TRY(q.add(cpart, splits, 1, 256, 0, 0, gr.views_b[0], 128, 1, 128));
        TRY(q.add(cpart, splits, 1, 256, 0, kSigmaChannel, gr.alpha_b, 1, 1, 1));
        TRY(q.add(part, splits, 256, 256, 0, 0, gr.views_w[0], ldv, 128, 256));
        TRY(q.add(part, splits, 256, 256, kSigmaChannel, 0, gr.alpha_w, 256, 1, 256));
    }
    TRY(run_tn(q, w.dV0, 256, 128, act(kActDir), 64, 64, Pp, gr.views_w[0] + IDN_W, ldv, 128, IDN_VIEWS_CH, s));
    for (int l = 7; l >= 1; --l) {
        const float* cur = w.dA[l];
        if (l == 5) {
            TRY(run_tn(q, cur, 256, 256, a_l(5), 256, 256, Pp, gr.pts_w[5] + IDN_PTS_CH + C, ld5, 256, 256, s, gr.pts_b[5], 256));
            TRY(run_tn(q, cur, 256, 256, act(kActX0), 64, 64, Pp, gr.pts_w[5], ld5, 256, IDN_PTS_CH, s));
        } else {
            TRY(run_tn(q, cur, 256, 256, a_l(l), 256, 256, Pp, gr.pts_w[l], 256, 256, 256, s, gr.pts_b[l], 256));
        }
    }
    TRY(run_tn(q, w.dA[0], 256, 256, act(kActX0), 64, 64, Pp, gr.pts_w[0], ld0, 256, IDN_PTS_CH, s, gr.pts_b[0], 256));
    TRY(q.flush(s));
#undef TRY
    {
        FoldBwdArgs f{p, aud, expr, latent, gr.pts_b[0], gr.pts_b[5], gr.views_b[0], gr.pts_w[0], gr.pts_w[5],
                      gr.views_w[0], d_aud, d_latent, d_expr};
        const int total = IDN_W * C + (IDN_W / 2) * p.dim_expr + C * 64;
        if (total > 0) {
            hipLaunchKernelGGL(fold_bwd_kernel, dim3((total + 255) / 256), dim3(256), 0, s, f);
            IDN_HIP_CHECK(hipGetLastError());
        }
    }
    return IDN_OK;
}

int launch_pass_bwd(const idn_facenerf_params& p, const idn_facenerf_grads& gr, const float* aud, const float* expr,
                    const float* latent, const float* acts, const float* raw, const float* z, const float* rays,
                    const float* bc, int64_t n_rays, int S, const float* g_rgb, const float* g_fg, const float* g_lw,
                    const float* g_acc, float* d_aud, float* d_latent, void* ws_, size_t ws_bytes, hipStream_t s) {
    const int64_t P = n_rays * S;
    const int64_t Pp = (P + 127) / 128 * 128;
    if (S < 2 || S > 256) return fail(IDN_EUNSUPPORTED, "pass_bwd: n_samples %d outside [2, 256]", S);
    const BwdWs w = carve_bwd(reinterpret_cast<char*>(ws_), Pp);
    if (!ws_ || ws_bytes < w.bytes) return fail(IDN_EWORKSPACE, "backward workspace %zu < %zu", ws_bytes, w.bytes);

    IDN_HIP_CHECK(hipMemsetAsync(w.dRGB, 0, (size_t)Pp * 64 * 4, s));
    if (Pp > P) IDN_HIP_CHECK(hipMemsetAsync(w.dV0 + (size_t)P * 256, 0, (size_t)(Pp - P) * 256 * 4, s));
    {
        CompBwdArgs a{reinterpret_cast<const float4*>(raw), z, rays, bc, g_rgb, g_fg, g_lw, g_acc,
                      w.dRGB, 64, w.dV0 + kSigmaChannel, 256, (long)n_rays, S};
        const dim3 grid((unsigned)((n_rays + 3) / 4)), block(256);
        switch ((S + 63) / 64) {
            case 1: hipLaunchKernelGGL(composite_bwd_kernel<1>, grid, block, 0, s, a); break;
            case 2: hipLaunchKernelGGL(composite_bwd_kernel<2>, grid, block, 0, s, a); break;
            case 3: hipLaunchKernelGGL(composite_bwd_kernel<3>, grid, block, 0, s, a); break;
            default: hipLaunchKernelGGL(composite_bwd_kernel<4>, grid, block, 0, s, a); break;
        }
        IDN_HIP_CHECK(hipGetLastError());
    }
    return bwd_tail(p, gr, aud, expr, latent, acts, Pp, w, d_aud, nullptr, d_latent, s);
}

__global__ __launch_bounds__(256) void head_seed_kernel(const float* g_out, long n, long p_pad, float* d_rgb, float* dv0) {
    const long idx = (long)blockIdx.x * 256 + threadIdx.x;
    const long p = idx >> 4;
    const int q = (int)(idx & 15);
    if (p >= p_pad) return;
    f32x4 v = {0.f, 0.f, 0.f, 0.f};
    if (q == 0 && p < n) v = f32x4{g_out[p * 4 + 0], g_out[p * 4 + 1], g_out[p * 4 + 2], 0.f};
    *reinterpret_cast<f32x4*>(d_rgb + p * 64 + 4 * q) = v;
    if (q == 0) dv0[p * 256 + kSigmaChannel] = p < n ? g_out[p * 4 + 3] : 0.f;
}

constexpr int kDxFrags = 2 * 64 + 16;
constexpr int kDxLds = kDxFrags * kFragBytes;
constexpr int kDxWaves = 16;
static_assert(kDxLds <= 160 * 1024, "the fragments must fit a CU's LDS");
struct DxArgs {
    const float* w0; int ld0;
    const float* w5; int ld5;
    const float* wv; int ldv;
    const float* dA0; const float* dA5; const float* dV0;
    long n, p_pad;
    float* d_x;
};
__global__ __launch_bounds__(64 * kDxWaves, 1) void dx_kernel(DxArgs a) {
    extern __shared__ __attribute__((aligned(16))) f32x4 dx_frag[];
    const int tid = threadIdx.x, lane = tid & 63;
    const int wave = __builtin_amdgcn_readfirstlane(tid >> 6);
    const int j = lane & 31, hh = lane >> 5;
    for (int e = tid; e < kDxFrags * 64; e += 64 * kDxWaves) {
        const int f = e >> 6, i = e & 31, h = (e >> 5) & 1;
        float v[4];
        for (int t = 0; t < 4; ++t) {
            if (f < 128) {
                const int g = f >> 1, col = 32 * (f & 1) + i, k = 8 * g + 4 * h + t;
                const float* row = k < IDN_W ? a.w0 + (long)k * a.ld0 : a.w5 + (long)(k - IDN_W) * a.ld5;
                v[t] = col < IDN_PTS_CH ? row[col] : 0.f;
            } else {
                const int k = 8 * (f - 128) + 4 * h + t;
                v[t] = i < IDN_VIEWS_CH ? a.wv[(long)k * a.ldv + IDN_W + i] : 0.f;
            }
        }
        dx_frag[e] = f32x4{v[0], v[1], v[2], v[3]};
    }
    __syncthreads();
    const long ntiles = a.p_pad / 32;
    for (long tile = (long)blockIdx.x * kDxWaves + wave; tile < ntiles; tile += (long)gridDim.x * kDxWaves) {
        const long p = tile * 32 + j;
        f32x16 acc0, acc1, accv;
        for (int r = 0; r < 16; ++r) acc0[r] = acc1[r] = accv[r] = 0.f;
        const float* r0 = a.dA0 + p * 256 + 4 * hh;
        const float* r5 = a.dA5 + p * 256 + 4 * hh;
        const float* rv = a.dV0 + p * 256 + 4 * hh;
#pragma unroll 4
        for (int g = 0; g < 32; ++g) {
            const f32x4 d = *reinterpret_cast<const f32x4*>(r0 + 8 * g);
            const f32x4 w0 = dx_frag[(2 * g) * 64 + lane], w1 = dx_frag[(2 * g + 1) * 64 + lane];
#pragma unroll
            for (int t = 0; t < 4; ++t) {
                acc0 = mfma32(w0[t], d[t], acc0);
                acc1 = mfma32(w1[t], d[t], acc1);
            }
        }
#pragma unroll 4
        for (int g = 0; g < 32; ++g) {
            const f32x4 d = *reinterpret_cast<const f32x4*>(r5 + 8 * g);
            const f32x4 w0 = dx_frag[(64 + 2 * g) * 64 + lane], w1 = dx_frag[(64 + 2 * g + 1) * 64 + lane];
#pragma unroll
            for (int t = 0; t < 4; ++t) {
                acc0 = mfma32(w0[t], d[t], acc0);
                acc1 = mfma32(w1[t], d[t], acc1);
            }
        }
#pragma unroll 4
        for (int g = 0; g < 16; ++g) {
            const f32x4 d = *reinterpret_cast<const f32x4*>(rv + 8 * g);
            const f32x4 w = dx_frag[(128 + g) * 64 + lane];
#pragma unroll
            for (int t = 0; t < 4; ++t) accv = mfma32(w[t], d[t], accv);
        }
        if (p < a.n) {
            float* o = a.d_x + p * (IDN_PTS_CH + IDN_VIEWS_CH);
#pragma unroll
            for (int r = 0; r < 16; ++r) {
                const int col = d_row(r, hh);
                o[col] = acc0[r];
                if (col < IDN_PTS_CH - 32) o[32 + col] = acc1[r];
                if (col < IDN_VIEWS_CH) o[IDN_PTS_CH + col] = accv[r];
            }
        }
    }
}

int launch_facenerf_bwd(const idn_facenerf_params& p, const idn_facenerf_grads& gr, const float* aud, const float* expr,
                        const float* latent, const float* acts, int64_t n, const float* g_out, float* d_x, float* d_aud,
                        float* d_expr, float* d_latent, void* ws_, size_t ws_bytes, hipStream_t s) {
    const int64_t Pp = (n + 127) / 128 * 128;
    const BwdWs w = carve_bwd(reinterpret_cast<char*>(ws_), Pp);
    if (!ws_ || ws_bytes < w.bytes) return fail(IDN_EWORKSPACE, "backward workspace %zu < %zu", ws_bytes, w.bytes);
    {
        const long threads = (long)Pp * 16;
        hipLaunchKernelGGL(head_seed_kernel, dim3((unsigned)((threads + 255) / 256)), dim3(256), 0, s, g_out, (long)n, (long)Pp,
                           w.dRGB, w.dV0);
        IDN_HIP_CHECK(hipGetLastError());
    }
    if (int e = bwd_tail(p, gr, aud, expr, latent, acts, Pp, w, d_aud, d_expr, d_latent, s)) return e;
    if (d_x) {
        static LaunchSetup setup;
        int num_cu = 0;
        if (int e = setup.get([]() -> int {
                IDN_HIP_CHECK(hipFuncSetAttribute(reinterpret_cast<const void*>(&dx_kernel), hipFuncAttributeMaxDynamicSharedMemorySize, kDxLds));
                return IDN_OK;
            }, &num_cu))
            return e;
        const int C = p.dim_aud + p.dim_expr + p.dim_latent;
        const DxArgs da{p.pts_w[0], IDN_PTS_CH + C, p.pts_w[5], IDN_PTS_CH + C + IDN_W, p.views_w[0], IDN_W + IDN_VIEWS_CH + p.dim_expr,
                        w.dA[0], w.dA[5], w.dV0, (long)n, (long)Pp, d_x};
        const int64_t groups = (Pp / 32 + kDxWaves - 1) / kDxWaves;
        const int grid = (int)(groups < num_cu ? groups : num_cu);
        hipLaunchKernelGGL(dx_kernel, dim3(grid), dim3(64 * kDxWaves), kDxLds, s, da);
        IDN_HIP_CHECK(hipGetLastError());
    }
    return IDN_OK;
}


}
```

Measured before the change: 129.1 million.

## Skip 32-point blocks with zero upstream gradient in the backward pass

Measured after the change: 129.5 million (median of 6 runs). No clear change (+0.3%).

```diff
diff --git a/ideal-nerf_amd/csrc/idn_internal.h b/ideal-nerf_amd/csrc/idn_internal.h
--- a/ideal-nerf_amd/csrc/idn_internal.h
+++ b/ideal-nerf_amd/csrc/idn_internal.h
@@ -185,12 +185,22 @@
 constexpr int kBwdNumSlices = kBwdStreamFrags / kSliceFrags;
 
 int launch_pack_f32_bwd(const idn_facenerf_params& p, float* packed_bwd, hipStream_t s);
+struct BwdBlockList {
+    const int* list;
+    const int* count;
+    float* dump;
+};
+__device__ __forceinline__ int scalar_load_i32(const int* p) {
+    int v;
+    asm volatile("s_load_dword %0, %1, 0x0\n\ts_waitcnt lgkmcnt(0)" : "=&s"(v) : "s"(p) : "memory");
+    return v;
+}
 int launch_delta_chain(const float* packed_bwd, const float* acts, int64_t p_pad, const float* d_rgb, float* dv0,
-                       float* dv2, float* dv1, float* const da[8], hipStream_t s);
+                       float* dv2, float* dv1, float* const da[8], const BwdBlockList& bl, hipStream_t s);
 size_t bwd_stream_floats_x6();
 int launch_pack_bf16x6_bwd(const idn_facenerf_params& p, float* packed_bwd, hipStream_t s);
 int launch_delta_chain_x6(const float* packed_bwd, const float* acts, int64_t p_pad, const float* d_rgb, float* dv0,
-                          float* dv2, float* dv1, float* const da[8], hipStream_t s);
+                          float* dv2, float* dv1, float* const da[8], const BwdBlockList& bl, hipStream_t s);
 size_t bwd_workspace_bytes(int64_t n_points);
 size_t dw_gemm_workspace_bytes();
 int launch_dw_gemm(const float* delta, int ld_delta, const float* acts, int ld_acts, int64_t rows, float* dW, float* db, int pipe,
diff --git a/ideal-nerf_amd/csrc/mlp_f32_bwd.hip b/ideal-nerf_amd/csrc/mlp_f32_bwd.hip
--- a/ideal-nerf_amd/csrc/mlp_f32_bwd.hip
+++ b/ideal-nerf_amd/csrc/mlp_f32_bwd.hip
@@ -67,6 +67,9 @@
     float* dv2;
     float* dv1;
     float* da[8];
+    const int* list;
+    const int* count;
+    float* dump;
 };
 
 template <int F0, int NT, int KG, bool LAST, class BGet, class Side>
@@ -205,12 +208,18 @@
     FragReader fr;
     fr.addr0 = (uint32_t)(uintptr_t)(__attribute__((address_space(3))) char*)ring + lane * 16;
     fr.addr1 = fr.addr0 + 64 * kFragBytes;
-    const long ntiles = a.p_pad >> 7;
+    const int cnt = scalar_load_i32(a.count);
+    const int rounds = (cnt + 3) >> 2;
     const uint32_t raddr = (uint32_t)(uintptr_t)(__attribute__((address_space(3))) float*)stage + (h * kStagePitch + m) * 4;
 
-    for (long tile = blockIdx.x; tile < ntiles; tile += gridDim.x) {
-        const long p0 = tile * 128 + wave * 32;
+    for (int tile = blockIdx.x; tile < rounds; tile += gridDim.x) {
+        int ent = tile * 4 + wave;
+        const bool spare = ent >= cnt;
+        if (spare) ent = cnt - 1;
+        const long blk = scalar_load_i32(a.list + ent);
+        const long p0 = blk * 32;
         const long P = p0 + m;
+        const long s0 = spare ? 0 : p0;
         const f32x4 drgb = *reinterpret_cast<const f32x4*>(a.d_rgb + P * 64);
         const float dsig = a.dv0[P * 256 + kSigmaChannel];
 
@@ -218,7 +227,7 @@
         float rb[4];
         typedef uint32_t u32x4 __attribute__((ext_vector_type(4)));
         const u32x4* mbase = reinterpret_cast<const u32x4*>(a.acts + (size_t)kActCols * a.p_pad);
-        auto mask_load = [&](int id) { return mbase[mask_index(id, a.p_pad, tile * 4 + wave, lane)]; };
+        auto mask_load = [&](int id) { return mbase[mask_index(id, a.p_pad, blk, lane)]; };
         u32x4 mask_nxt = mask_load(10);
         auto tiles_get = [](f32x16* arr) {
             return [arr](auto G, auto J) {
@@ -234,7 +243,7 @@
             const u32x4 mv = mask_nxt;
             const uint32_t mk[4] = {mv.x, mv.y, mv.z, mv.w};
             if (next_id >= 0) mask_nxt = mask_load(next_id);
-            const MaskSide<NT, KG / 2, LD> side{&out[0], mk, rows_rsrc(dst + p0 * LD, LD), (uint32_t)((h * LD + m) * 4), stage, rb, raddr, m, h};
+            const MaskSide<NT, KG / 2, LD> side{&out[0], mk, rows_rsrc((spare ? a.dump : dst) + s0 * LD, LD), (uint32_t)((h * LD + m) * 4), stage, rb, raddr, m, h};
             run_stage<F0, NT, KG, decltype(LASTc)::value != 0>(out, bget, ws, fr, side);
             side.finish();
         };
@@ -271,7 +280,7 @@
 }
 
 int launch_delta_chain(const float* packed_bwd, const float* acts, int64_t p_pad, const float* d_rgb, float* dv0,
-                       float* dv2, float* dv1, float* const da[8], hipStream_t s) {
+                       float* dv2, float* dv1, float* const da[8], const BwdBlockList& bl, hipStream_t s) {
     if (p_pad <= 0) return IDN_OK;
     if (p_pad % 128) return fail(IDN_EINVAL, "delta chain: p_pad %lld is not a multiple of 128", (long long)p_pad);
     static LaunchSetup setup;
@@ -284,7 +293,7 @@
         return e;
     const int64_t ntiles = p_pad / 128;
     const int grid = (int)(ntiles < num_cu ? ntiles : num_cu);
-    DeltaArgs a{packed_bwd, acts, (long)p_pad, d_rgb, dv0, dv2, dv1, {}};
+    DeltaArgs a{packed_bwd, acts, (long)p_pad, d_rgb, dv0, dv2, dv1, {}, bl.list, bl.count, bl.dump};
     for (int l = 0; l < 8; ++l) a.da[l] = da[l];
     ProfScope prof(s, p_pad, IDN_PROF_DELTA_CHAIN);
     hipLaunchKernelGGL(delta_chain_kernel, dim3(grid), dim3(256), kDeltaLds, s, a);
@@ -448,11 +457,17 @@
     FragReader fr;
     fr.addr0 = (uint32_t)(uintptr_t)(__attribute__((address_space(3))) char*)ring + lane * 16;
     fr.addr1 = fr.addr0 + 64 * kFragBytes;
-    const long ntiles = a.p_pad >> 7;
+    const int cnt = scalar_load_i32(a.count);
+    const int rounds = (cnt + 3) >> 2;
     f32x4 pref[3] = {{0.f, 0.f, 0.f, 0.f}, {0.f, 0.f, 0.f, 0.f}, {0.f, 0.f, 0.f, 0.f}};
 
-    for (long tile = blockIdx.x; tile < ntiles; tile += gridDim.x) {
-        const long P = tile * 128 + wave * 32 + m;
+    for (int tile = blockIdx.x; tile < rounds; tile += gridDim.x) {
+        int ent = tile * 4 + wave;
+        const bool spare = ent >= cnt;
+        if (spare) ent = cnt - 1;
+        const long blk = scalar_load_i32(a.list + ent);
+        const long P = blk * 32 + m;
+        const long Ps = spare ? m : P;
         const f32x4 drgb = *reinterpret_cast<const f32x4*>(a.d_rgb + P * 64);
         const float dsig = a.dv0[P * 256 + kSigmaChannel];
         f32x4 in_rgb[3], in_sig[3];
@@ -480,7 +495,7 @@
         f32x16 O[8];
         typedef uint32_t u32x4 __attribute__((ext_vector_type(4)));
         const u32x4* mbase = reinterpret_cast<const u32x4*>(a.acts + (size_t)kActCols * a.p_pad);
-        auto mask_load = [&](int id) { return mbase[mask_index(id, a.p_pad, tile * 4 + wave, lane)]; };
+        auto mask_load = [&](int id) { return mbase[mask_index(id, a.p_pad, blk, lane)]; };
         u32x4 mask_nxt = mask_load(10);
         auto tiles = [&](auto Q, auto S_) {
             constexpr int q = decltype(Q)::value, s = decltype(S_)::value;
@@ -491,7 +506,7 @@
             const u32x4 mv = mask_nxt;
             const uint32_t mk[4] = {mv.x, mv.y, mv.z, mv.w};
             if (next_id >= 0) mask_nxt = mask_load(next_id);
-            const MaskStoreSide<decltype(KSc)::value> side{O, mk, dst + P * LD + 4 * h};
+            const MaskStoreSide<decltype(KSc)::value> side{O, mk, (spare ? a.dump : dst) + Ps * LD + 4 * h};
             constexpr bool trunk = decltype(F0c)::value >= bwd6_f0(4);
             run_stage6<decltype(F0c)::value, NT, decltype(KSc)::value, decltype(LASTc)::value != 0, decltype(YOUNGERc)::value, (trunk ? 4 : 0)>(O, bget, ws, fr, pref, side);
             if constexpr (trunk) side.whole(ic<NT - 1>{});
@@ -522,7 +537,7 @@
 }
 
 int launch_delta_chain_x6(const float* packed_bwd, const float* acts, int64_t p_pad, const float* d_rgb, float* dv0,
-                          float* dv2, float* dv1, float* const da[8], hipStream_t s) {
+                          float* dv2, float* dv1, float* const da[8], const BwdBlockList& bl, hipStream_t s) {
     if (p_pad <= 0) return IDN_OK;
     if (p_pad % 128) return fail(IDN_EINVAL, "delta chain: p_pad %lld is not a multiple of 128", (long long)p_pad);
     static LaunchSetup setup;
@@ -535,7 +550,7 @@
         return e;
     const int64_t ntiles = p_pad / 128;
     const int grid = (int)(ntiles < num_cu ? ntiles : num_cu);
-    DeltaArgs a{packed_bwd, acts, (long)p_pad, d_rgb, dv0, dv2, dv1, {}};
+    DeltaArgs a{packed_bwd, acts, (long)p_pad, d_rgb, dv0, dv2, dv1, {}, bl.list, bl.count, bl.dump};
     for (int l = 0; l < 8; ++l) a.da[l] = da[l];
     ProfScope prof(s, p_pad, IDN_PROF_DELTA_CHAIN_X6);
     hipLaunchKernelGGL(x6::delta_chain_x6_kernel, dim3(grid), dim3(256), x6::kDelta6Lds, s, a);
diff --git a/ideal-nerf_amd/csrc/train.hip b/ideal-nerf_amd/csrc/train.hip
--- a/ideal-nerf_amd/csrc/train.hip
+++ b/ideal-nerf_amd/csrc/train.hip
@@ -21,6 +21,8 @@
     int chunks_per_split;
     float* cpart;
     int b_split, b_off0, b_off1;
+    const int* list;
+    const int* count;
 };
 
 template <int N>
@@ -99,47 +101,96 @@
         for (int b = 0; b < KTW; ++b)
             for (int r = 0; r < 16; ++r) acc[a][b][r] = 0.f;
 
-    const long c_begin = (long)split * g.chunks_per_split;
-    long c_end = c_begin + g.chunks_per_split;
-    const long c_total = g.P / R;
+    const bool has_list = g.list != nullptr;
+    const long c_total = has_list ? (long)scalar_load_i32(g.count) * 32 / R : g.P / R;
+    const int cps = has_list ? (int)((c_total + gridDim.z - 1) / gridDim.z) : g.chunks_per_split;
+    const long c_begin = (long)split * cps;
+    long c_end = c_begin + cps;
     if (c_end > c_total) c_end = c_total;
+    auto chunk_rows = [&](long cc, int& r0, int& r1) {
+        if (!has_list) {
+            r0 = (int)(cc * R);
+            r1 = r0 + 32;
+        } else if constexpr (R == 16) {
+            r0 = scalar_load_i32(g.list + (cc >> 1)) * 32 + (int)(cc & 1) * 16;
+            r1 = r0;
+        } else if constexpr (R == 32) {
+            r0 = scalar_load_i32(g.list + cc) * 32;
+            r1 = r0;
+        } else {
+            static_assert(R == 16 || R == 32 || R == 64, "chunks of a half, one or two 32-row blocks");
+            r0 = scalar_load_i32(g.list + 2 * cc) * 32;
+            r1 = scalar_load_i32(g.list + 2 * cc + 1) * 32;
+        }
+    };
     const bool colsum_block = g.cpart != nullptr && blockIdx.y == 0;
     const bool do_colsum = colsum_block && tid < BN;
     const int ccol = tid < BN ? tid : 0;
     float csum = 0.0f;
 
     constexpr int kRowsPerPieceA = 256 / BN > 0 ? 256 / BN : 1, kRowsPerPieceB = 256 / BK > 0 ? 256 / BK : 1;
-    const __amdgpu_buffer_rsrc_t rsrcA = __builtin_amdgcn_make_buffer_rsrc(const_cast<float*>(g.A + n0 + c_begin * R * (long)g.lda), 0, 0xfffffffc, 0x00020000);
-    const __amdgpu_buffer_rsrc_t rsrcB = __builtin_amdgcn_make_buffer_rsrc(const_cast<float*>(g.B + k0 + c_begin * R * (long)g.ldb), 0, 0xfffffffc, 0x00020000);
+    auto write_out = [&]() {
+        if (do_colsum) g.cpart[(long)split * g.N + n0 + tid] = csum;
+        float* out = g.part + (long)split * g.N * g.K;
+#pragma unroll
+        for (int x = 0; x < NTW; ++x)
+#pragma unroll
+            for (int r = 0; r < 16; ++r) {
+                const int n = n0 + NTW * (32 * wr + d_row(r, hh)) + x;
+                float* dst = out + (long)n * g.K + k0 + KTW * (32 * wc + i);
+                if constexpr (KTW == 4) {
+                    *reinterpret_cast<f32x4*>(dst) = f32x4{acc[x][0][r], acc[x][1][r], acc[x][2][r], acc[x][3][r]};
+                } else {
+#pragma unroll
+                    for (int y = 0; y < KTW; ++y) dst[y] = acc[x][y][r];
+                }
+            }
+    };
+    if (c_begin >= c_end) {
+        write_out();
+        return;
+    }
+    int row0, row0b;
+    chunk_rows(c_begin, row0, row0b);
+    const __amdgpu_buffer_rsrc_t rsrcA = __builtin_amdgcn_make_buffer_rsrc(const_cast<float*>(g.A + n0 + row0 * (long)g.lda), 0, 0xfffffffc, 0x00020000);
+    const __amdgpu_buffer_rsrc_t rsrcB = __builtin_amdgcn_make_buffer_rsrc(const_cast<float*>(g.B + k0 + row0 * (long)g.ldb), 0, 0xfffffffc, 0x00020000);
     const uint32_t voffA = ((lane / (BN / 4)) * g.lda + (lane % (BN / 4)) * 4) * 4;
     const uint32_t voffB = ((lane / (BK / 4)) * g.ldb + (lane % (BK / 4)) * 4) * 4;
     const uint32_t rowA = g.lda * 4, rowB = g.ldb * 4;
-    auto piece_a = [&](long c, int buf, int ja) {
+    auto piece_row = [&](int q0, int q1, int r) { return (R > 32 && r >= 32) ? q1 + (r - 32) : q0 + r; };
+    auto piece_a = [&](int q0, int q1, int buf, int ja) {
         const int pc = NPA * w + ja;
         __builtin_amdgcn_raw_ptr_buffer_load_lds(rsrcA, (__attribute__((address_space(3))) void*)(tn_smem + buf * kTileFloats + pc * 256), 16, voffA,
-                                                 (uint32_t)(((c - c_begin) * R + pc * kRowsPerPieceA) * rowA), 0, 0);
+                                                 (uint32_t)piece_row(q0, q1, pc * kRowsPerPieceA) * rowA, 0, 0);
     };
-    auto piece_b = [&](long c, int buf, int jb) {
+    auto piece_b = [&](int q0, int q1, int buf, int jb) {
         const int pc = NPB * w + jb;
         __builtin_amdgcn_raw_ptr_buffer_load_lds(rsrcB, (__attribute__((address_space(3))) void*)(tn_smem + buf * kTileFloats + R * BN + pc * 256), 16, voffB,
-                                                 (uint32_t)(((c - c_begin) * R + pc * kRowsPerPieceB) * rowB), 0, 0);
+                                                 (uint32_t)piece_row(q0, q1, pc * kRowsPerPieceB) * rowB, 0, 0);
     };
-    auto piece = [&](long c, int buf, int j) {
-        if (j < NPA) piece_a(c, buf, j);
-        else if (j < NP) piece_b(c, buf, j - NPA);
+    auto piece = [&](int q0, int q1, int buf, int j) {
+        if (j < NPA) piece_a(q0, q1, buf, j);
+        else if (j < NP) piece_b(q0, q1, buf, j - NPA);
     };
     const uint32_t smem0 = (uint32_t)(uintptr_t)(__attribute__((address_space(3))) float*)tn_smem;
     const uint32_t a_addr0 = smem0 + (hh * BN + NTW * (32 * wr + i)) * 4;
     const uint32_t b_addr0 = smem0 + (R * BN + hh * BK + KTW * (32 * wc + i)) * 4;
-    for (int ahead = 0; ahead < NB - 1; ++ahead)
-        for (int j = 0; j < NP; ++j) piece(c_begin + ahead < c_end ? c_begin + ahead : c_end - 1, ahead, j);
+    for (int ahead = 0; ahead < NB - 1; ++ahead) {
+        int q0, q1;
+        chunk_rows(c_begin + ahead < c_end ? c_begin + ahead : c_end - 1, q0, q1);
+        for (int j = 0; j < NP; ++j) piece(q0 - row0, q1 - row0, ahead, j);
+    }
     int buf = 0;
     for (long c = c_begin; c < c_end; ++c) {
+        const long cnext = c + NB - 1 < c_end ? c + NB - 1 : c_end - 1;
+        int nq0, nq1;
+        chunk_rows(cnext, nq0, nq1);
+        nq0 -= row0;
+        nq1 -= row0;
         asm volatile("s_waitcnt vmcnt(%0)" ::"n"((NB - 2) * NP) : "memory");
         __builtin_amdgcn_s_barrier();
         asm volatile("" ::: "memory");
         const int buf2 = buf >= 1 ? buf - 1 : NB - 1;
-        const long cnext = c + NB - 1 < c_end ? c + NB - 1 : c_end - 1;
         float cs[16];
         auto cs_issue = [&](int batch) {
             const uint32_t caddr = smem0 + buf * (kTileFloats * 4) + ccol * 4 + batch * (16 * BN * 4);
@@ -176,7 +227,7 @@
             for (int it = 0; it < kSteps / 4; ++it) {
                 step(a0v, b0v,
                      [&]() { a1v.template issue<kStepA>(pa); b1v.template issue<kStepB>(pb); },
-                     [&]() { if (2 * it < NPA) piece_a(cnext, buf2, 2 * it); },
+                     [&]() { if (2 * it < NPA) piece_a(nq0, nq1, buf2, 2 * it); },
                      [&]() {
                          if (colsum_block && it < R / 16) {
                              tn_static_for<16>([&](auto Row) { csum += landed(cs[decltype(Row)::value]); });
@@ -186,7 +237,7 @@
                      });
                 step(a1v, b1v,
                      [&]() { a0v.template issue<0>(pa); b0v.template issue<0>(pb); },
-                     [&]() { if (2 * it + 1 < NPA) piece_a(cnext, buf2, 2 * it + 1); },
+                     [&]() { if (2 * it + 1 < NPA) piece_a(nq0, nq1, buf2, 2 * it + 1); },
                      [&]() { if (colsum_block && it + 1 < R / 16) cs_issue(it + 1); });
             }
 #pragma unroll 1
@@ -194,14 +245,14 @@
                 const bool last = it == kSteps / 4 - 1;
                 step(a0v, b0v,
                      [&]() { a1v.template issue<kStepA>(pa); b1v.template issue<kStepB>(pb); },
-                     [&]() { if (2 * it < NPB) piece_b(cnext, buf2, 2 * it); },
+                     [&]() { if (2 * it < NPB) piece_b(nq0, nq1, buf2, 2 * it); },
                      [&]() {
                          pa = last ? pa : pa + 2 * kStepA;
                          pb = last ? pb : pb + 2 * kStepB;
                      });
                 step(a1v, b1v,
                      [&]() { a0v.template issue<0>(pa); b0v.template issue<0>(pb); },
-                     [&]() { if (2 * it + 1 < NPB) piece_b(cnext, buf2, 2 * it + 1); },
+                     [&]() { if (2 * it + 1 < NPB) piece_b(nq0, nq1, buf2, 2 * it + 1); },
                      [&]() {});
             }
         } else {
@@ -240,22 +291,22 @@
 #pragma unroll 1
             for (int it = 0; it < kSteps / 8; ++it) {
                 quad(a0v, b0v, a1v, b1v, a2v, b2v, a3v, b3v, false,
-                     [&]() { if (2 * it < NPA) piece_a(cnext, buf2, 2 * it); },
+                     [&]() { if (2 * it < NPA) piece_a(nq0, nq1, buf2, 2 * it); },
                      [&]() {
                          if (colsum_block && it < R / 16) {
                              tn_static_for<16>([&](auto Row) { csum += landed(cs[decltype(Row)::value]); });
                          }
                      });
                 quad(a2v, b2v, a3v, b3v, a0v, b0v, a1v, b1v, false,
-                     [&]() { if (2 * it + 1 < NPA) piece_a(cnext, buf2, 2 * it + 1); },
+                     [&]() { if (2 * it + 1 < NPA) piece_a(nq0, nq1, buf2, 2 * it + 1); },
                      [&]() { if (colsum_block && it + 1 < R / 16) cs_issue(it + 1); });
             }
 #pragma unroll 1
             for (int it = 0; it < kSteps / 8; ++it) {
                 quad(a0v, b0v, a1v, b1v, a2v, b2v, a3v, b3v, false,
-                     [&]() { if (2 * it < NPB) piece_b(cnext, buf2, 2 * it); }, [&]() {});
+                     [&]() { if (2 * it < NPB) piece_b(nq0, nq1, buf2, 2 * it); }, [&]() {});
                 quad(a2v, b2v, a3v, b3v, a0v, b0v, a1v, b1v, it == kSteps / 8 - 1,
-                     [&]() { if (2 * it + 1 < NPB) piece_b(cnext, buf2, 2 * it + 1); }, [&]() {});
+                     [&]() { if (2 * it + 1 < NPB) piece_b(nq0, nq1, buf2, 2 * it + 1); }, [&]() {});
             }
             lds_retire<0>(a1v, b1v);
         }
@@ -263,21 +314,7 @@
         buf = buf + 1 == NB ? 0 : buf + 1;
     }
     asm volatile("s_waitcnt vmcnt(0)" ::: "memory");
-    if (do_colsum) g.cpart[(long)split * g.N + n0 + tid] = csum;
-    float* out = g.part + (long)split * g.N * g.K;
-#pragma unroll
-    for (int x = 0; x < NTW; ++x)
-#pragma unroll
-        for (int r = 0; r < 16; ++r) {
-            const int n = n0 + NTW * (32 * wr + d_row(r, hh)) + x;
-            float* dst = out + (long)n * g.K + k0 + KTW * (32 * wc + i);
-            if constexpr (KTW == 4) {
-                *reinterpret_cast<f32x4*>(dst) = f32x4{acc[x][0][r], acc[x][1][r], acc[x][2][r], acc[x][3][r]};
-            } else {
-#pragma unroll
-                for (int y = 0; y < KTW; ++y) dst[y] = acc[x][y][r];
-            }
-        }
+    write_out();
 }
 
 typedef __bf16 tn_bf16x8 __attribute__((ext_vector_type(8)));
@@ -313,29 +350,47 @@
     asm volatile("s_waitcnt lgkmcnt(%3)" : "+v"(f[0].v), "+v"(f[1].v), "+v"(f[2].v) : "n"(N) : "memory");
 }
 
-__device__ __forceinline__ void gemm_tn_x6_item(const TNArgs& g, const int split, char* x6_smem) {
+__device__ __forceinline__ void gemm_tn_x6_item(const TNArgs& g, const int split, const int splits, char* x6_smem) {
     const int tid = threadIdx.x, lane = tid & 63;
     const int w = __builtin_amdgcn_readfirstlane(tid >> 6);
     const int i = lane & 31, hh = lane >> 5;
     const int wr = w >> 1, wc = w & 1;
+
+    const bool has_list = g.list != nullptr;
+    const long c_total = has_list ? 2L * scalar_load_i32(g.count) : g.P / kTnRows;
+    const int cps = has_list ? (int)((c_total + splits - 1) / splits) : g.chunks_per_split;
+    const long c_begin = (long)split * cps;
+    long c_end = c_begin + cps;
+    if (c_end > c_total) c_end = c_total;
+    const int n_chunks = (int)(c_end - c_begin);
+    if (n_chunks <= 0) {
+        f32x4* out4 = reinterpret_cast<f32x4*>(g.part + (long)split * g.N * g.K);
+        for (int e = tid; e < g.N * g.K / 4; e += 256) out4[e] = f32x4{0.f, 0.f, 0.f, 0.f};
+        if (g.cpart != nullptr) g.cpart[(long)split * g.N + tid] = 0.0f;
+        return;
+    }
     f32x16 acc[4][4];
 #pragma unroll
     for (int a = 0; a < 4; ++a)
 #pragma unroll
         for (int b = 0; b < 4; ++b)
             for (int r = 0; r < 16; ++r) acc[a][b][r] = 0.f;
-
-    const long c_begin = (long)split * g.chunks_per_split;
-    long c_end = c_begin + g.chunks_per_split;
-    const long c_total = g.P / kTnRows;
-    if (c_end > c_total) c_end = c_total;
-    const int n_chunks = (int)(c_end - c_begin);
+    auto vchunk = [&](int k) { return c_begin + (k < n_chunks ? k : n_chunks - 1); };
+    auto row_of = [&](int block, long v) { return block * 32 + (int)(v & 1) * kTnRows; };
+    auto block_now = [&](long v) { return has_list ? scalar_load_i32(g.list + (v >> 1)) : (int)(v >> 1); };
+    const int row0 = row_of(block_now(c_begin), c_begin);
+    auto rel_now = [&](int k) {
+        const long v = vchunk(k);
+        return row_of(block_now(v), v) - row0;
+    };
+    const int rel1 = rel_now(1);
+    int nbase = rel_now(2), block_nxt = 0;
     auto make_rsrc = [](const float* ptr) {
         const uint64_t a64 = (uint64_t)(uintptr_t)ptr;
         return tn_i32x4{(int)(uint32_t)a64, (int)((uint32_t)(a64 >> 32) & 0xffffu), (int)0xfffffffcu, 0x00020000};
     };
-    const tn_i32x4 rsrcA = make_rsrc(g.A + c_begin * kTnRows * (long)g.lda);
-    const tn_i32x4 rsrcB = make_rsrc(g.B + c_begin * kTnRows * (long)g.ldb);
+    const tn_i32x4 rsrcA = make_rsrc(g.A + row0 * (long)g.lda);
+    const tn_i32x4 rsrcB = make_rsrc(g.B + row0 * (long)g.ldb);
     const int voff = tid * 4;
     const int voffB = g.b_split ? (tid < 128 ? g.b_off0 : g.b_off1) + (tid & 127) * 4 : voff;
     const int rowA = g.lda * 4, rowB = g.ldb * 4;
@@ -346,8 +401,7 @@
         asm volatile("buffer_load_dword %0, %1, %2, %3 offen" : "+v"(dst) : "v"(vo), "s"(rsrc), "s"(soff) : "memory");
     };
     auto load_row = [&](float& dst, const tn_i32x4& rsrc, int soff) { load_row_at(dst, rsrc, soff, voff); };
-    auto load_chunk = [&](int rc) {
-        const int base = (rc < n_chunks ? rc : n_chunks - 1) * kTnRows;
+    auto load_chunk = [&](int base) {
 #pragma unroll
         for (int p = 0; p < kTnRows; ++p) load_row(ra[p], rsrcA, (base + p) * rowA);
 #pragma unroll
@@ -383,7 +437,7 @@
     colsum();
     split_store(0, 0, ra);
     split_store(0, 1, rb);
-    load_chunk(1);
+    load_chunk(rel1);
     asm volatile("s_waitcnt lgkmcnt(0)" ::: "memory");
     __builtin_amdgcn_s_barrier();
     asm volatile("" ::: "memory");
@@ -430,7 +484,8 @@
         x6_retire<0>(fa[2]);
         x6_retire<0>(fa[3]);
         const unsigned live_mask = rc + 1 < n_chunks ? 0xffffffffu : 0u;
-        const int nbase = (rc + 2 < n_chunks ? rc + 2 : n_chunks - 1) * kTnRows;
+        const long v3 = vchunk(rc + 3);
+        asm volatile("s_load_dword %0, %1, 0x0" : "=&s"(block_nxt) : "s"(has_list ? g.list + (v3 >> 1) : reinterpret_cast<const int*>(g.A)) : "memory");
         char* const dst = my_slot + (buf ^ 1) * kX6BufBytes;
         unsigned pw[2][3][8];
         float t0 = 0.f, t1 = 0.f;
@@ -484,9 +539,10 @@
             if constexpr (k < kX1) slice(ic_<0>{}, ic_<k>{});
             else slice(ic_<1>{}, ic_<k - kX1>{});
             if constexpr (k == 59) {
-                asm volatile("s_waitcnt lgkmcnt(0)" ::: "memory");
+                asm volatile("s_waitcnt lgkmcnt(0)" : "+s"(block_nxt)::"memory");
                 __builtin_amdgcn_s_barrier();
                 asm volatile("" ::: "memory");
+                nbase = row_of(has_list ? block_nxt : (int)(v3 >> 1), v3) - row0;
                 issue_first_row(a_base + (buf ^ 1) * kX6BufBytes, b_base + (buf ^ 1) * kX6BufBytes);
             }
             __builtin_amdgcn_sched_barrier(0);
@@ -516,7 +572,7 @@
     extern __shared__ __attribute__((aligned(16))) char x6_smem[];
     const int item = __builtin_amdgcn_readfirstlane((int)blockIdx.z / b.splits);
     const int split = __builtin_amdgcn_readfirstlane((int)blockIdx.z - item * b.splits);
-    gemm_tn_x6_item(b.it[item], split, x6_smem);
+    gemm_tn_x6_item(b.it[item], split, b.splits, x6_smem);
 }
 
 constexpr int kMaxReduceItems = 32;
@@ -574,6 +630,7 @@
     float* d_rgb; int ld_rgb;
     float* d_sig; int ld_sig;
     long n_rays; int S;
+    unsigned char* flags;
 };
 
 template <int SPL>
@@ -675,6 +732,7 @@
             a.d_rgb[p * a.ld_rgb + 0] = d0;
             a.d_rgb[p * a.ld_rgb + 1] = d1;
             a.d_rgb[p * a.ld_rgb + 2] = d2;
+            if (dsig != 0.f || d0 != 0.f || d1 != 0.f || d2 != 0.f) a.flags[p >> 5] = 1;
         }
     }
 }
@@ -746,8 +804,43 @@
 
 struct BwdWs {
     float *dA[8], *dV[2], *dV0, *dRGB, *part, *cpart, *wbwd;
+    unsigned char* flags;
+    int* list;
+    int* count;
+    float* dump;
     size_t bytes;
-};
+    BwdBlockList block_list() const { return BwdBlockList{list, count, dump}; }
+};
+
+__global__ __launch_bounds__(1024) void block_list_kernel(const unsigned char* flags, int nb, int dense, int* list, int* count) {
+    __shared__ int sums[1024];
+    __shared__ int first_off;
+    const int t = threadIdx.x;
+    const int per = (nb + 1023) / 1024;
+    const int b0 = t * per < nb ? t * per : nb, b1 = b0 + per < nb ? b0 + per : nb;
+    int n = 0, off = nb;
+    for (int b = b1 - 1; b >= b0; --b) {
+        const bool on = dense || flags[b] != 0;
+        n += on ? 1 : 0;
+        if (!on) off = b;
+    }
+    if (t == 0) first_off = nb;
+    sums[t] = n;
+    __syncthreads();
+    atomicMin(&first_off, off);
+    for (int d = 1; d < 1024; d <<= 1) {
+        const int v = t >= d ? sums[t - d] : 0;
+        __syncthreads();
+        sums[t] += v;
+        __syncthreads();
+    }
+    const int total = sums[1023];
+    const int extra = (total & 1) ? first_off : -1;
+    int at = sums[t] - n + (extra >= 0 && extra < b0 ? 1 : 0);
+    for (int b = b0; b < b1; ++b)
+        if (dense || flags[b] != 0 || b == extra) list[at++] = b;
+    if (t == 0) count[0] = total + (extra >= 0 ? 1 : 0);
+}
 static BwdWs carve_bwd(char* base, int64_t p_pad) {
     BwdWs w;
     size_t off = 0;
@@ -761,9 +854,14 @@
     w.dV[1] = w.dV[0] + 128;
     w.dV0 = take((size_t)p_pad * 256);
     w.dRGB = take((size_t)p_pad * 64);
+    const size_t nb = (size_t)(p_pad / 32);
+    w.flags = reinterpret_cast<unsigned char*>(take((nb + 3) / 4));
     w.part = take((size_t)kMaxSplits * kPartFloatsPerSplit);
     w.cpart = take((size_t)kColsumBlocks * 256 * kGemmsPerPass);
     w.wbwd = take(bwd_stream_floats_x6());
+    w.list = reinterpret_cast<int*>(take(nb));
+    w.count = reinterpret_cast<int*>(take(64));
+    w.dump = take(32 * 256);
     w.bytes = off;
     return w;
 }
@@ -782,6 +880,13 @@
     return v;
 }
 static int default_gemm_pipe() { return env_pipe_f32() ? kPipeF32 : kPipeX6; }
+static int env_skip_zero_blocks() {
+    static const int v = [] {
+        const char* e = getenv("IDN_BWD_SKIP_ZERO_BLOCKS");
+        return (e && e[0] == '0' && e[1] == 0) ? 0 : 1;
+    }();
+    return v;
+}
 struct X6Pending {
     TNBatch b;
     int splits = 0;
@@ -833,8 +938,8 @@
     IDN_HIP_CHECK(hipGetLastError());
     return IDN_OK;
 }
-static int run_tn_partials(X6Pending& x6, const float* A, int lda, int N, const float* B, int ldb, int K, int64_t P, float* part,
-                           int* splits_out, hipStream_t s, float* cpart = nullptr, int pipe = -1, const float* B2 = nullptr) {
+static int run_tn_partials(X6Pending& x6, const BwdBlockList& bl, const float* A, int lda, int N, const float* B, int ldb, int K, int64_t P,
+                           float* part, int* splits_out, hipStream_t s, float* cpart = nullptr, int pipe = -1, const float* B2 = nullptr) {
     if (pipe < 0) pipe = default_gemm_pipe();
     if (B2 && !(N == 256 && K == 256 && pipe == kPipeX6)) return fail(IDN_EINVAL, "gemm_tn: a split B needs the 256 x 256 bf16-piece kernel");
     int ntw, ktw;
@@ -861,7 +966,7 @@
     if (splits < 1) splits = 1;
     const int cps = (int)((chunks + splits - 1) / splits);
     splits = (int)((chunks + cps - 1) / cps);
-    TNArgs g{A, lda, B, ldb, part, N, K, (long)P, cps, cpart, 0, 0, 0};
+    TNArgs g{A, lda, B, ldb, part, N, K, (long)P, cps, cpart, 0, 0, 0, bl.list, bl.count};
     if (B2) {
         const float* base = B < B2 ? B : B2;
         const int64_t o0 = (int64_t)(B - base) * 4, o1 = (int64_t)(B2 - base) * 4;
@@ -895,7 +1000,9 @@
     float* part_next;
     float* cpart_next;
     X6Pending x6;
-    ReduceQueue(float* part_pool, float* cpart_pool, int expected_x6_items = 1) : part_next(part_pool), cpart_next(cpart_pool) {
+    BwdBlockList bl;
+    ReduceQueue(float* part_pool, float* cpart_pool, int expected_x6_items = 1, BwdBlockList rows = BwdBlockList{nullptr, nullptr, nullptr})
+        : part_next(part_pool), cpart_next(cpart_pool), bl(rows) {
         b.n = 0;
         x6.expected_items = expected_x6_items;
     }
@@ -919,7 +1026,7 @@
                     const float** part_out, const float** cpart_out, bool colsum, hipStream_t s, int pipe, const float* B2 = nullptr) {
     float* part = q.part_next;
     float* cpart = colsum ? q.cpart_next : nullptr;
-    if (int e = run_tn_partials(q.x6, A, lda, N, B, ldb, K, P, part, splits, s, cpart, pipe, B2)) return e;
+    if (int e = run_tn_partials(q.x6, q.bl, A, lda, N, B, ldb, K, P, part, splits, s, cpart, pipe, B2)) return e;
     q.part_next += (size_t)(*splits) * N * K;
     if (colsum) q.cpart_next += (size_t)(*splits) * N;
     *part_out = part;
@@ -962,14 +1069,20 @@
     auto a_l = [&](int l) { return act(kActA1 + l - 1); };
     auto v_l = [&](int l) { return act(kActV1 + l - 1); };
 #define TRY(x) do { if (int e_ = (x)) return e_; } while (0)
+    {
+        const int dense = (!env_skip_zero_blocks() || (uint64_t)Pp * 1024u >= ((uint64_t)1 << 32)) ? 1 : 0;
+        hipLaunchKernelGGL(block_list_kernel, dim3(1), dim3(1024), 0, s, w.flags, (int)(Pp / 32), dense, w.list, w.count);
+        IDN_HIP_CHECK(hipGetLastError());
+    }
+    const BwdBlockList bl = w.block_list();
     if (!env_pipe_f32()) {
         TRY(launch_pack_bf16x6_bwd(p, w.wbwd, s));
-        TRY(launch_delta_chain_x6(w.wbwd, acts, Pp, w.dRGB, w.dV0, w.dV[0], w.dV[1], w.dA, s));
+        TRY(launch_delta_chain_x6(w.wbwd, acts, Pp, w.dRGB, w.dV0, w.dV[0], w.dV[1], w.dA, bl, s));
     } else {
         TRY(launch_pack_f32_bwd(p, w.wbwd, s));
-        TRY(launch_delta_chain(w.wbwd, acts, Pp, w.dRGB, w.dV0, w.dV[0], w.dV[1], w.dA, s));
-    }
-    ReduceQueue q(w.part, w.cpart, kX6ItemsPerPass);
+        TRY(launch_delta_chain(w.wbwd, acts, Pp, w.dRGB, w.dV0, w.dV[0], w.dV[1], w.dA, bl, s));
+    }
+    ReduceQueue q(w.part, w.cpart, kX6ItemsPerPass, bl);
     TRY(run_tn(q, w.dRGB, 64, 64, v_l(3), 128, 128, Pp, gr.rgb_w, 128, 3, 128, s, gr.rgb_b, 3));
     const int pipe = default_gemm_pipe();
     if (pipe == kPipeX6) {
@@ -1028,11 +1141,11 @@
     const BwdWs w = carve_bwd(reinterpret_cast<char*>(ws_), Pp);
     if (!ws_ || ws_bytes < w.bytes) return fail(IDN_EWORKSPACE, "backward workspace %zu < %zu", ws_bytes, w.bytes);
 
-    IDN_HIP_CHECK(hipMemsetAsync(w.dRGB, 0, (size_t)Pp * 64 * 4, s));
+    IDN_HIP_CHECK(hipMemsetAsync(w.dRGB, 0, (size_t)(reinterpret_cast<char*>(w.flags) + Pp / 32 - reinterpret_cast<char*>(w.dRGB)), s));
     if (Pp > P) IDN_HIP_CHECK(hipMemsetAsync(w.dV0 + (size_t)P * 256, 0, (size_t)(Pp - P) * 256 * 4, s));
     {
         CompBwdArgs a{reinterpret_cast<const float4*>(raw), z, rays, bc, g_rgb, g_fg, g_lw, g_acc,
-                      w.dRGB, 64, w.dV0 + kSigmaChannel, 256, (long)n_rays, S};
+                      w.dRGB, 64, w.dV0 + kSigmaChannel, 256, (long)n_rays, S, w.flags};
         const dim3 grid((unsigned)((n_rays + 3) / 4)), block(256);
         switch ((S + 63) / 64) {
             case 1: hipLaunchKernelGGL(composite_bwd_kernel<1>, grid, block, 0, s, a); break;
@@ -1045,7 +1158,7 @@
     return bwd_tail(p, gr, aud, expr, latent, acts, Pp, w, d_aud, nullptr, d_latent, s);
 }
 
-__global__ __launch_bounds__(256) void head_seed_kernel(const float* g_out, long n, long p_pad, float* d_rgb, float* dv0) {
+__global__ __launch_bounds__(256) void head_seed_kernel(const float* g_out, long n, long p_pad, float* d_rgb, float* dv0, unsigned char* flags) {
     const long idx = (long)blockIdx.x * 256 + threadIdx.x;
     const long p = idx >> 4;
     const int q = (int)(idx & 15);
@@ -1053,7 +1166,11 @@
     f32x4 v = {0.f, 0.f, 0.f, 0.f};
     if (q == 0 && p < n) v = f32x4{g_out[p * 4 + 0], g_out[p * 4 + 1], g_out[p * 4 + 2], 0.f};
     *reinterpret_cast<f32x4*>(d_rgb + p * 64 + 4 * q) = v;
-    if (q == 0) dv0[p * 256 + kSigmaChannel] = p < n ? g_out[p * 4 + 3] : 0.f;
+    if (q == 0) {
+        const float dsig = p < n ? g_out[p * 4 + 3] : 0.f;
+        dv0[p * 256 + kSigmaChannel] = dsig;
+        if (dsig != 0.f || v[0] != 0.f || v[1] != 0.f || v[2] != 0.f) flags[p >> 5] = 1;
+    }
 }
 
 constexpr int kDxFrags = 2 * 64 + 16;
@@ -1067,6 +1184,8 @@
     const float* dA0; const float* dA5; const float* dV0;
     long n, p_pad;
     float* d_x;
+    const int* list;
+    const int* count;
 };
 __global__ __launch_bounds__(64 * kDxWaves, 1) void dx_kernel(DxArgs a) {
     extern __shared__ __attribute__((aligned(16))) f32x4 dx_frag[];
@@ -1089,8 +1208,9 @@
         dx_frag[e] = f32x4{v[0], v[1], v[2], v[3]};
     }
     __syncthreads();
-    const long ntiles = a.p_pad / 32;
-    for (long tile = (long)blockIdx.x * kDxWaves + wave; tile < ntiles; tile += (long)gridDim.x * kDxWaves) {
+    const long ntiles = *a.count;
+    for (long t = (long)blockIdx.x * kDxWaves + wave; t < ntiles; t += (long)gridDim.x * kDxWaves) {
+        const long tile = a.list[t];
         const long p = tile * 32 + j;
         f32x16 acc0, acc1, accv;
         for (int r = 0; r < 16; ++r) acc0[r] = acc1[r] = accv[r] = 0.f;
@@ -1145,8 +1265,9 @@
     if (!ws_ || ws_bytes < w.bytes) return fail(IDN_EWORKSPACE, "backward workspace %zu < %zu", ws_bytes, w.bytes);
     {
         const long threads = (long)Pp * 16;
+        IDN_HIP_CHECK(hipMemsetAsync(w.flags, 0, (size_t)(Pp / 32), s));
         hipLaunchKernelGGL(head_seed_kernel, dim3((unsigned)((threads + 255) / 256)), dim3(256), 0, s, g_out, (long)n, (long)Pp,
-                           w.dRGB, w.dV0);
+                           w.dRGB, w.dV0, w.flags);
         IDN_HIP_CHECK(hipGetLastError());
     }
     if (int e = bwd_tail(p, gr, aud, expr, latent, acts, Pp, w, d_aud, d_expr, d_latent, s)) return e;
@@ -1160,7 +1281,8 @@
             return e;
         const int C = p.dim_aud + p.dim_expr + p.dim_latent;
         const DxArgs da{p.pts_w[0], IDN_PTS_CH + C, p.pts_w[5], IDN_PTS_CH + C + IDN_W, p.views_w[0], IDN_W + IDN_VIEWS_CH + p.dim_expr,
-                        w.dA[0], w.dA[5], w.dV0, (long)n, (long)Pp, d_x};
+                        w.dA[0], w.dA[5], w.dV0, (long)n, (long)Pp, d_x, w.list, w.count};
+        if (n > 0) IDN_HIP_CHECK(hipMemsetAsync(d_x, 0, (size_t)n * (IDN_PTS_CH + IDN_VIEWS_CH) * 4, s));
         const int64_t groups = (Pp / 32 + kDxWaves - 1) / kDxWaves;
         const int grid = (int)(groups < num_cu ? groups : num_cu);
         hipLaunchKernelGGL(dx_kernel, dim3(grid), dim3(64 * kDxWaves), kDxLds, s, da);
```
